# SCZwangxiao/video-ReTaKe

Measured on NVIDIA B200. Metric: 2048-frame DPSelect+PivotKV frames/s, higher is better.
Workload: dtype bf16

## Files before the change

include/rtk_b200.h:

```cpp
#ifndef RTK_B200_H_
#define RTK_B200_H_

#include <stddef.h>
#include <stdint.h>

#ifdef __cplusplus
extern "C" {
#endif

#define RTK_ABI_VERSION 3

#define RTK_E_BADARG      (-1)
#define RTK_E_ALIGN       (-2)
#define RTK_E_UNSUPPORTED (-3)
#define RTK_E_WORKSPACE   (-4)
#define RTK_E_DRIVER      (-5)

int         rtk_version(void);
const char* rtk_build_id(void);
const char* rtk_error_string(int code);
int         rtk_debug_key_elision(int on);
int64_t     rtk_launch_count(void);


int rtk_dpselect_dis(const void* x, int64_t T, int64_t N, int64_t C, int halo, float* dis, void* stream);

int rtk_dpselect_select(const float* dis, int64_t T, int64_t N, int64_t t, int sync,
                        int32_t* idx, uint8_t* mask, void* stream);

int rtk_dpselect_gather(const void* x, int64_t T, int64_t N, int64_t C, const int32_t* idx, int64_t t,
                        int sync, void* out, void* stream);

int rtk_dpselect_keyframe(const void* x, int64_t T, int64_t N, int64_t C, int64_t t, int sync, float* dis,
                          int32_t* idx, uint8_t* mask, void* out, void* stream);

int rtk_dpselect_gather_owned(const void* x_local, int64_t frames_local, int64_t frame_first, int64_t t0, int64_t t1,
                              int64_t N, int64_t C, const int32_t* idx, int64_t t, int sync, void* out, void* stream);

int rtk_gather_rows(const void* x, int64_t row_bytes, const int64_t* src_row, int64_t rows, void* out, void* stream);

size_t rtk_mallm_workspace_bytes(int64_t T, int64_t N, int64_t C, int hard);
int rtk_mallm_compress(const void* x, const void* sizes_in, int64_t T, int64_t N, int64_t C, int64_t t, int sync, int hard,
                       void* out, void* sizes_out, void* workspace, size_t workspace_bytes, void* stream);


int rtk_pivot_rope(const void* x, int64_t heads, int64_t L, int64_t D, int64_t stride_h, int64_t stride_l,
                   const void* cos, const void* sin, int n_pos, const int32_t* mrope_section_host,
                   float inv_scale2, int forward, void* out, int64_t out_stride_h, int64_t out_stride_l,
                   void* stream);

size_t rtk_pivot_score_workspace_bytes(int64_t H, int64_t L);

int rtk_pivot_score(const void* q, int64_t H, int64_t q_stride_h, int64_t q_stride_l,
                    const void* k, int64_t KVH, int64_t k_stride_h, int64_t k_stride_l,
                    int64_t L, int64_t D, void* head_scores, void* workspace, size_t workspace_bytes,
                    void* stream);

int rtk_pivot_select(const void* head_scores, int64_t KVH, int64_t L, const uint8_t* keymask, int64_t keep,
                     int32_t* keep_idx, void* score_out, void* stream);

int rtk_pivot_compact(const void* k, const void* v, int64_t KVH, int64_t L, int64_t D,
                      int64_t stride_h, int64_t stride_l, const int32_t* keep_idx, int64_t keep,
                      void* k_out, void* v_out, int64_t out_stride_h,
                      const int64_t* pos, int n_pos, int64_t* pos_out, int reforge, void* stream);

int rtk_kv_block_copy(int n_jobs, const void* const* src, void* const* dst, const int64_t* heads, const int64_t* rows,
                      const int64_t* src_stride_h, const int64_t* src_stride_l, const int64_t* dst_stride_h,
                      const int64_t* dst_stride_l, int64_t D, void* stream);

int rtk_pivot_rope_tables(const int64_t* pos, int n_pos, int64_t L, int64_t D, const float* inv_freq,
                          const int32_t* mrope_section_host, float attention_scaling, void* cos_out, void* sin_out,
                          void* stream);

typedef struct rtk_pivot_update_args {
    const void* q; int64_t H, q_stride_h, q_stride_l;
    const void* k; int64_t KVH, k_stride_h, k_stride_l;
    const void* v; int64_t v_stride_h, v_stride_l;
    int64_t k_stride_h_in, k_stride_l_in;
    int64_t L, D;
    const uint8_t* keymask;
    int64_t keep;
    int32_t reforge;
    int32_t n_pos;
    const int64_t* pos;
    const void* cos; const void* sin;
    const float* inv_freq;
    float attention_scaling, inv_scale2;
    int32_t mrope_section[3];
    int32_t skip_select;
    void* k_out; void* v_out; int64_t out_stride_h;
    int64_t* pos_out;
    int32_t* keep_idx;
    void* head_scores;
    void* workspace; size_t workspace_bytes;
    void* ev_score_begin; void* ev_score_end;
    int64_t pos_out_stride;
    int32_t skip_score;
    int32_t score_rows;
    int32_t xchg_world, xchg_rank;
    uint32_t xchg_epoch;
    void* xchg_scores[8];
    uint32_t* xchg_flags[8];
} rtk_pivot_update_args;

size_t rtk_pivot_update_workspace_bytes(int64_t H, int64_t KVH, int64_t L, int64_t D);
int rtk_pivot_update(const rtk_pivot_update_args* args, void* stream);

size_t rtk_pivot_update_batch_workspace_bytes(int64_t H, int64_t KVH, int64_t L, int64_t D, int64_t n_layers);
int rtk_pivot_update_batch(const rtk_pivot_update_args* layers, int64_t n_layers, void* workspace, size_t workspace_bytes,
                           void* stream);

#ifdef __cplusplus
}
#endif
#endif
```

video-retake_b200/csrc/pivot_misc.cu:

```cuda
#include <climits>

#include <stdlib.h>

#include "rtk_common.cuh"

namespace rtk {

struct RopeParams {
    int heads, L, D, n_pos, forward;
    long long stride_h, stride_l, out_stride_h, out_stride_l;
    int heads2;
    const __nv_bfloat16* x2;
    __nv_bfloat16* out2;
    long long stride_h2, stride_l2, out_stride_h2, out_stride_l2;
    int bound[6];
    float inv_scale2;
};

static bool mrope_bounds(int n_pos, const int32_t* sec, int64_t D, int bound[6]) {
    int acc = 0;
    for (int i = 0; i < 6; ++i) {
        acc += n_pos == 3 ? sec[i % 3] : 0;
        bound[i] = acc;
    }
    return n_pos != 3 || acc == D;
}

__device__ __forceinline__ int rope_pos_row(const RopeParams& p, int c) {
    if (p.n_pos == 1) return 0;
    int i = 0;
    while (i < 5 && c >= p.bound[i]) ++i;
    return i % 3;
}

__global__ void __launch_bounds__(256)
pivot_rope_table_kernel(const long long* __restrict__ pos, const float* __restrict__ inv_freq, RopeParams p, float scaling,
                        __nv_bfloat16* __restrict__ cos_t, __nv_bfloat16* __restrict__ sin_t) {
    pdl_enter();
    const int half = p.D >> 1;
    const long long total = (long long)p.L * p.D;
    for (long long i = (long long)blockIdx.x * blockDim.x + threadIdx.x; i < total; i += (long long)gridDim.x * blockDim.x) {
        const int c = (int)(i % p.D);
        const int l = (int)(i / p.D);
        const long long pv = pos[(size_t)rope_pos_row(p, c) * p.L + l];
        const float ang = inv_freq[c < half ? c : c - half] * (float)pv;
        cos_t[i] = __float2bfloat16_rn(cosf(ang) * scaling);
        sin_t[i] = __float2bfloat16_rn(sinf(ang) * scaling);
    }
}

__device__ __forceinline__ void rope_rotate_pair(float xa, float xb, float cosa, float sina, float cosb, float sinb, int forward,
                                                 float inv_scale2, __nv_bfloat16& oa, __nv_bfloat16& ob) {
    const float ta = round_bf16(xa * cosa), ra = round_bf16(-xb * sina);
    const float tb = round_bf16(xb * cosb), rb = round_bf16(xa * sinb);
    float ya, yb;
    if (forward) {
        ya = ta + ra;
        yb = tb + rb;
    } else {
        ya = round_bf16(ta - ra) * inv_scale2;
        yb = round_bf16(tb - rb) * inv_scale2;
    }
    oa = __float2bfloat16_rn(ya);
    ob = __float2bfloat16_rn(yb);
}

__device__ __forceinline__ void rope_table_entry(const RopeParams& p, const float* __restrict__ inv_freq, const long long* pv,
                                                 int c, float scaling, float& co, float& si) {
    const int half = p.D >> 1;
    const float ang = inv_freq[c < half ? c : c - half] * (float)pv[rope_pos_row(p, c)];
    co = __bfloat162float(__float2bfloat16_rn(cosf(ang) * scaling));
    si = __bfloat162float(__float2bfloat16_rn(sinf(ang) * scaling));
}

#ifndef RTK_UNROPE_TOK
#define RTK_UNROPE_TOK 2
#endif
constexpr int kUnropeTok = RTK_UNROPE_TOK;

__device__ __forceinline__ uint32_t sub_bf16x2_rn(uint32_t a, uint32_t b) {
    uint32_t d;
    asm("sub.rn.bf16x2 %0, %1, %2;" : "=r"(d) : "r"(a), "r"(b));
    return d;
}
__device__ __forceinline__ uint32_t add_bf16x2_rn(uint32_t a, uint32_t b) {
    uint32_t d;
    asm("add.rn.bf16x2 %0, %1, %2;" : "=r"(d) : "r"(a), "r"(b));
    return d;
}
__device__ __forceinline__ void unrotate_bf16x2(uint32_t xa, uint32_t xb, uint32_t cs, uint32_t sn, bool scale, float inv_scale2,
                                                uint32_t& oa, uint32_t& ob) {
    const uint32_t ta = mul_bf16x2_rn(xa, cs), ra = mul_bf16x2_rn(xb ^ 0x80008000u, sn);
    const uint32_t tb = mul_bf16x2_rn(xb, cs), rb = mul_bf16x2_rn(xa, sn);
    oa = sub_bf16x2_rn(ta, ra);
    ob = sub_bf16x2_rn(tb, rb);
    if (scale) {
        oa = scale_bf16x2_rn(oa, inv_scale2);
        ob = scale_bf16x2_rn(ob, inv_scale2);
    }
}

__device__ __forceinline__ void unrope_qk_body(const __nv_bfloat16* __restrict__ x, const long long* __restrict__ pos,
                                               const float* __restrict__ inv_freq, float scaling,
                                               __nv_bfloat16* __restrict__ out, const RopeParams& p) {
    __shared__ __align__(16) __nv_bfloat16 s_cos[kUnropeTok][128], s_sin[kUnropeTok][128];
    const int half = p.D >> 1;
    const int vec_per_row = half >> 3;
    const int ntask = (p.heads + p.heads2) * vec_per_row;
    const int tid = threadIdx.x;
    const bool scale = p.inv_scale2 != 1.0f;
    const int v0 = tid % vec_per_row, h0 = tid / vec_per_row;
    const bool second0 = h0 >= p.heads;
    const long long src_h0 = second0 ? (long long)(h0 - p.heads) * p.stride_h2 : (long long)h0 * p.stride_h;
    const long long src_l0 = second0 ? p.stride_l2 : p.stride_l;
    const __nv_bfloat16* src0 = (second0 ? p.x2 : x) + src_h0 + v0 * 8;
    for (int l0 = blockIdx.x * kUnropeTok; l0 < p.L; l0 += gridDim.x * kUnropeTok) {
        const int nl = min(kUnropeTok, p.L - l0);
        uint4 lo4[kUnropeTok], hi4[kUnropeTok];
        if (tid < ntask) {
#pragma unroll
            for (int t = 0; t < kUnropeTok; ++t) {
                if (t < nl) {
                    lo4[t] = *reinterpret_cast<const uint4*>(src0 + (l0 + t) * src_l0);
                    hi4[t] = *reinterpret_cast<const uint4*>(src0 + (l0 + t) * src_l0 + half);
                }
            }
        }
        for (int e = tid; e < nl * half; e += blockDim.x) {
            const int t = e / half, c = e - t * half;
            long long pv[3] = {0, 0, 0};
            for (int r = 0; r < p.n_pos; ++r) pv[r] = pos[(size_t)r * p.L + l0 + t];
            float co, si;
            rope_table_entry(p, inv_freq, pv, c, scaling, co, si);
            s_cos[t][c] = __float2bfloat16_rn(co);
            s_sin[t][c] = __float2bfloat16_rn(si);
        }
        __syncthreads();
#pragma unroll
        for (int t = 0; t < kUnropeTok; ++t) {
            if (t >= nl) break;
            const int l = l0 + t;
            for (int task = tid; task < ntask; task += blockDim.x) {
                const int v = task % vec_per_row, h = task / vec_per_row;
                const int c0 = v * 8;
                const bool second = h >= p.heads;
                const __nv_bfloat16* src = second ? p.x2 + (h - p.heads) * p.stride_h2 + l * p.stride_l2 : x + h * p.stride_h + l * p.stride_l;
                __nv_bfloat16* dst = second ? p.out2 + (h - p.heads) * p.out_stride_h2 + l * p.out_stride_l2
                                            : out + h * p.out_stride_h + l * p.out_stride_l;
                uint4 a4 = lo4[t], b4 = hi4[t];
                if (task != tid) {
                    a4 = *reinterpret_cast<const uint4*>(src + c0);
                    b4 = *reinterpret_cast<const uint4*>(src + c0 + half);
                }
                const uint4 cs = *reinterpret_cast<const uint4*>(&s_cos[t][c0]);
                const uint4 sn = *reinterpret_cast<const uint4*>(&s_sin[t][c0]);
                uint4 ol4, oh4;
                unrotate_bf16x2(a4.x, b4.x, cs.x, sn.x, scale, p.inv_scale2, ol4.x, oh4.x);
                unrotate_bf16x2(a4.y, b4.y, cs.y, sn.y, scale, p.inv_scale2, ol4.y, oh4.y);
                unrotate_bf16x2(a4.z, b4.z, cs.z, sn.z, scale, p.inv_scale2, ol4.z, oh4.z);
                unrotate_bf16x2(a4.w, b4.w, cs.w, sn.w, scale, p.inv_scale2, ol4.w, oh4.w);
                *reinterpret_cast<uint4*>(dst + c0) = ol4;
                *reinterpret_cast<uint4*>(dst + c0 + half) = oh4;
            }
        }
        __syncthreads();
    }
}

struct BatchLayers {
    const __nv_bfloat16* q[kMaxBatchLayers];
    const __nv_bfloat16* k[kMaxBatchLayers];
    const __nv_bfloat16* k_in[kMaxBatchLayers];
    const __nv_bfloat16* v[kMaxBatchLayers];
    __nv_bfloat16* qu[kMaxBatchLayers];
    __nv_bfloat16* ku[kMaxBatchLayers];
    const long long* pos[kMaxBatchLayers];
    const uint8_t* keymask[kMaxBatchLayers];
    __nv_bfloat16* k_out[kMaxBatchLayers];
    __nv_bfloat16* v_out[kMaxBatchLayers];
    long long* pos_out[kMaxBatchLayers];
    int32_t* keep_idx[kMaxBatchLayers];
    const __nv_bfloat16* head_scores[kMaxBatchLayers];
    long long q_stride_h[kMaxBatchLayers], q_stride_l[kMaxBatchLayers];
    long long kin_stride_h[kMaxBatchLayers], kin_stride_l[kMaxBatchLayers];
    long long k_stride_h[kMaxBatchLayers], k_stride_l[kMaxBatchLayers];
    long long v_stride_h[kMaxBatchLayers], v_stride_l[kMaxBatchLayers];
    long long out_stride_h[kMaxBatchLayers], pos_out_stride[kMaxBatchLayers];
};

__global__ void __launch_bounds__(256)
pivot_unrope_qk_batch_kernel(const __grid_constant__ BatchLayers t, const float* __restrict__ inv_freq, float scaling, RopeParams p) {
    pdl_enter();
    const int layer = blockIdx.y;
    p.stride_h = t.q_stride_h[layer]; p.stride_l = t.q_stride_l[layer];
    p.x2 = t.k_in[layer]; p.out2 = t.ku[layer];
    p.stride_h2 = t.kin_stride_h[layer]; p.stride_l2 = t.kin_stride_l[layer];
    unrope_qk_body(t.q[layer], t.pos[layer], inv_freq, scaling, t.qu[layer], p);
}

__global__ void __launch_bounds__(256)
pivot_rope_kernel(const __nv_bfloat16* __restrict__ x, const __nv_bfloat16* __restrict__ cos_t,
                  const __nv_bfloat16* __restrict__ sin_t, __nv_bfloat16* __restrict__ out, RopeParams p) {
    pdl_enter();
    const int half = p.D >> 1;
    const int vec_per_row = half >> 3;
    const long long total = (long long)(p.heads + p.heads2) * p.L * vec_per_row;
    for (long long i = (long long)blockIdx.x * blockDim.x + threadIdx.x; i < total; i += (long long)gridDim.x * blockDim.x) {
        const int v = (int)(i % vec_per_row);
        const long long hl = i / vec_per_row;
        const int l = (int)(hl % p.L);
        const int h = (int)(hl / p.L);
        const int c0 = v * 8;
        const bool second = h >= p.heads;
        const __nv_bfloat16* src = second ? p.x2 + (h - p.heads) * p.stride_h2 + l * p.stride_l2 : x + h * p.stride_h + l * p.stride_l;
        __nv_bfloat16* dst = second ? p.out2 + (h - p.heads) * p.out_stride_h2 + l * p.out_stride_l2
                                    : out + h * p.out_stride_h + l * p.out_stride_l;
        uint4 lo4 = *reinterpret_cast<const uint4*>(src + c0);
        uint4 hi4 = *reinterpret_cast<const uint4*>(src + c0 + half);
        const __nv_bfloat16* xl = reinterpret_cast<const __nv_bfloat16*>(&lo4);
        const __nv_bfloat16* xh = reinterpret_cast<const __nv_bfloat16*>(&hi4);
        uint4 ol4, oh4;
        __nv_bfloat16* ol = reinterpret_cast<__nv_bfloat16*>(&ol4);
        __nv_bfloat16* oh = reinterpret_cast<__nv_bfloat16*>(&oh4);
        const int rowa0 = rope_pos_row(p, c0), rowa1 = rope_pos_row(p, c0 + 7);
        const int rowb0 = rope_pos_row(p, c0 + half), rowb1 = rope_pos_row(p, c0 + half + 7);
        uint4 ca4, sa4, cb4, sb4;
        __nv_bfloat16* cav = reinterpret_cast<__nv_bfloat16*>(&ca4);
        __nv_bfloat16* sav = reinterpret_cast<__nv_bfloat16*>(&sa4);
        __nv_bfloat16* cbv = reinterpret_cast<__nv_bfloat16*>(&cb4);
        __nv_bfloat16* sbv = reinterpret_cast<__nv_bfloat16*>(&sb4);
        if (rowa0 == rowa1 && rowb0 == rowb1) {
            const size_t ia = ((size_t)rowa0 * p.L + l) * p.D + c0, ib = ((size_t)rowb0 * p.L + l) * p.D + c0 + half;
            ca4 = __ldg(reinterpret_cast<const uint4*>(cos_t + ia));
            sa4 = __ldg(reinterpret_cast<const uint4*>(sin_t + ia));
            cb4 = __ldg(reinterpret_cast<const uint4*>(cos_t + ib));
            sb4 = __ldg(reinterpret_cast<const uint4*>(sin_t + ib));
        } else {
#pragma unroll
            for (int e = 0; e < 8; ++e) {
                const int ca = c0 + e, cb = c0 + e + half;
                const size_t ia = ((size_t)rope_pos_row(p, ca) * p.L + l) * p.D + ca;
                const size_t ib = ((size_t)rope_pos_row(p, cb) * p.L + l) * p.D + cb;
                cav[e] = cos_t[ia]; sav[e] = sin_t[ia]; cbv[e] = cos_t[ib]; sbv[e] = sin_t[ib];
            }
        }
#pragma unroll
        for (int e = 0; e < 8; ++e)
            rope_rotate_pair(__bfloat162float(xl[e]), __bfloat162float(xh[e]), __bfloat162float(cav[e]), __bfloat162float(sav[e]),
                             __bfloat162float(cbv[e]), __bfloat162float(sbv[e]), p.forward, p.inv_scale2, ol[e], oh[e]);
        *reinterpret_cast<uint4*>(dst + c0) = ol4;
        *reinterpret_cast<uint4*>(dst + c0 + half) = oh4;
    }
}

bool key_elision_enabled();

struct KeyElide {
    const uint8_t* keymask[kMaxBatchLayers];
    int32_t* slot[kMaxBatchLayers];
    const __nv_bfloat16* k[kMaxBatchLayers];
    long long k_stride_h[kMaxBatchLayers], k_stride_l[kMaxBatchLayers];
    __nv_bfloat16* kc[kMaxBatchLayers];
    int32_t* n_keys;
    int L, KVH, D;
};

__global__ void __launch_bounds__(1024)
pivot_keymask_scan_kernel(const __grid_constant__ KeyElide e) {
    pdl_enter();
    __shared__ int wsum[32];
    const int layer = blockIdx.x, tid = threadIdx.x, lane = tid & 31, warp = tid >> 5;
    const uint8_t* __restrict__ m = e.keymask[layer];
    int32_t* __restrict__ slot = e.slot[layer];
    const int per = (e.L + 1023) / 1024;
    const int beg = min(tid * per, e.L), end = min(beg + per, e.L);
    int cnt = 0;
    for (int i = beg; i < end; ++i) cnt += !(m && m[i]);
    int inc = cnt;
#pragma unroll
    for (int o = 1; o < 32; o <<= 1) {
        const int n = __shfl_up_sync(0xffffffffu, inc, o);
        if (lane >= o) inc += n;
    }
    if (lane == 31) wsum[warp] = inc;
    __syncthreads();
    if (warp == 0) {
        const int w = wsum[lane];
        int winc = w;
#pragma unroll
        for (int o = 1; o < 32; o <<= 1) {
            const int n = __shfl_up_sync(0xffffffffu, winc, o);
            if (lane >= o) winc += n;
        }
        wsum[lane] = winc - w;
        if (lane == 31) e.n_keys[layer] = winc;
    }
    __syncthreads();
    int base = wsum[warp] + inc - cnt;
    for (int i = beg; i < end; ++i) slot[i] = (m && m[i]) ? -1 : base++;
}

__global__ void __launch_bounds__(256)
pivot_keys_compact_kernel(const __grid_constant__ KeyElide e) {
    pdl_enter();
    const int layer = blockIdx.y;
    const int vpr = e.D >> 3;
    const long long total = (long long)e.L * e.KVH * vpr;
    const int32_t* __restrict__ slot = e.slot[layer];
    for (long long i = (long long)blockIdx.x * blockDim.x + threadIdx.x; i < total; i += (long long)gridDim.x * blockDim.x) {
        const int v = (int)(i % vpr);
        const long long lh = i / vpr;
        const int h = (int)(lh % e.KVH);
        const int l = (int)(lh / e.KVH);
        const int sl = slot[l];
        if (sl < 0) continue;
        const uint4 w = __ldg(reinterpret_cast<const uint4*>(e.k[layer] + h * e.k_stride_h[layer] + l * e.k_stride_l[layer] + v * 8));
        *reinterpret_cast<uint4*>(e.kc[layer] + ((size_t)sl * e.KVH + h) * e.D + v * 8) = w;
    }
}

static int key_elide_prepare(KeyElide& ke, int n, ScoreBatch& sb, cudaStream_t st) {
    RTK_LAUNCH_PDL(pivot_keymask_scan_kernel, (unsigned)n, 1024, 0, st, ke);
    const long long total = (long long)ke.L * ke.KVH * (ke.D >> 3);
    long long gx = (total + 255) / 256;
    if (gx > 148 * 8) gx = 148 * 8;
    RTK_LAUNCH_PDL(pivot_keys_compact_kernel, dim3((unsigned)gx, (unsigned)n), 256, 0, st, ke);
    for (int i = 0; i < n; ++i) {
        sb.kc[i] = ke.kc[i];
        sb.slot[i] = ke.slot[i];
    }
    sb.n_keys = ke.n_keys;
    return 0;
}

static size_t key_elide_bytes(int64_t KVH, int64_t L, int64_t D) {
    return (((size_t)KVH * L * D * 2 + 255) & ~(size_t)255) + (((size_t)L * 4 + 255) & ~(size_t)255);
}

constexpr int kSelThreads = 1024;

__device__ void block_select_top(const uint32_t* keys, int L, int keep, int32_t* out_idx, int* sh ,
                                 int low_bit ) {
    const int tid = threadIdx.x, lane = tid & 31, warp = tid >> 5;
    const int per = (L + kSelThreads - 1) / kSelThreads;
    const int beg = min(tid * per, L), end = min(beg + per, L);
    uint32_t prefix = 0;
    for (int bit = 31; bit >= low_bit; --bit) {
        const uint32_t cand = prefix | (1u << bit);
        int cnt = 0;
        for (int i = beg; i < end; ++i) cnt += (keys[i] >= cand);
        cnt = __reduce_add_sync(0xffffffffu, cnt);
        int* buf = sh + 40 + 32 * (bit & 1);
        if (lane == 0) buf[warp] = cnt;
        __syncthreads();
        const int total = __reduce_add_sync(0xffffffffu, buf[lane]);
        if (total >= keep) prefix = cand;
    }
    __syncthreads();
    if (low_bit > 0 && (!(prefix & 0x80000000u) || (prefix >> low_bit) == (0xffffffffu >> low_bit)))
        prefix |= (1u << low_bit) - 1u;
    int gt = 0, eq = 0;
    for (int i = beg; i < end; ++i) { gt += (keys[i] > prefix); eq += (keys[i] == prefix); }
    auto block_excl_scan = [&](int v, int& total) {
        int inc = v;
#pragma unroll
        for (int o = 1; o < 32; o <<= 1) {
            const int n = __shfl_up_sync(0xffffffffu, inc, o);
            if (lane >= o) inc += n;
        }
        __syncthreads();
        if (lane == 31) sh[1 + warp] = inc;
        __syncthreads();
        if (warp == 0) {
            int w = sh[1 + lane], winc = w;
#pragma unroll
            for (int o = 1; o < 32; o <<= 1) {
                const int n = __shfl_up_sync(0xffffffffu, winc, o);
                if (lane >= o) winc += n;
            }
            sh[1 + lane] = winc - w;
            if (lane == 31) sh[33] = winc;
        }
        __syncthreads();
        total = sh[33];
        return sh[1 + warp] + inc - v;
    };
    int gt_total, eq_total;
    const int gt_before = block_excl_scan(gt, gt_total);
    const int eq_before = block_excl_scan(eq, eq_total);
    const int need = keep - gt_total;
    const int eq_taken_before = min(eq_before, need);
    int slot = gt_before + eq_taken_before;
    int eq_seen = eq_before;
    for (int i = beg; i < end; ++i) {
        const uint32_t k = keys[i];
        bool take = k > prefix;
        if (k == prefix) { take = eq_seen < need; ++eq_seen; }
        if (take) out_idx[slot++] = i;
    }
}

__device__ __forceinline__ void pivot_select_body(const __nv_bfloat16* __restrict__ head_scores, int KVH, int L,
                                                  const uint8_t* __restrict__ keymask, int keep, int32_t* __restrict__ keep_idx,
                                                  __nv_bfloat16* __restrict__ score_out, const long long* __restrict__ tpos,
                                                  long long* __restrict__ tmin_out) {
    extern __shared__ __align__(128) uint8_t smem[];
    uint32_t* keys = reinterpret_cast<uint32_t*>(smem);
    int* sh = reinterpret_cast<int*>(smem + (size_t)L * 4);
    const float rcp = 1.0f / (float)KVH;
    for (int i = threadIdx.x; i < L; i += blockDim.x) {
        float v[4] = {0.f, 0.f, 0.f, 0.f};
        for (int j = 0; j < KVH; ++j) v[j & 3] += __bfloat162float(head_scores[(size_t)j * L + i]);
        const __nv_bfloat16 s = __float2bfloat16_rn((((v[0] + v[1]) + v[2]) + v[3]) * rcp);
        if (score_out) score_out[i] = s;
        const float f = (keymask && keymask[i]) ? 1.0f : __bfloat162float(s);
        keys[i] = f32_to_ordered(f);
    }
    __syncthreads();
    block_select_top(keys, L, keep, keep_idx, sh, 16);
    if (tmin_out) {
        __syncthreads();
        long long* smin = reinterpret_cast<long long*>((reinterpret_cast<uintptr_t>(sh) + 7) & ~(uintptr_t)7);
        long long mn = LLONG_MAX;
        for (int j = threadIdx.x; j < keep; j += blockDim.x) mn = min(mn, tpos[keep_idx[j]]);
#pragma unroll
        for (int o = 16; o > 0; o >>= 1) mn = min(mn, __shfl_xor_sync(0xffffffffu, mn, o));
        if ((threadIdx.x & 31) == 0) smin[threadIdx.x >> 5] = mn;
        __syncthreads();
        if (threadIdx.x == 0) {
            for (int w = 1; w < (int)(blockDim.x >> 5); ++w) mn = min(mn, smin[w]);
            *tmin_out = mn;
        }
    }
}

__device__ __forceinline__ void st_release_sys(uint32_t* p, uint32_t v) {
    asm volatile("st.release.sys.global.u32 [%0], %1;" ::"l"(p), "r"(v) : "memory");
}
__device__ __forceinline__ uint32_t ld_acquire_sys(const uint32_t* p) {
    uint32_t v;
    asm volatile("ld.acquire.sys.global.u32 %0, [%1];" : "=r"(v) : "l"(p) : "memory");
    return v;
}
__device__ __forceinline__ unsigned long long globaltimer_ns() {
    unsigned long long t;
    asm volatile("mov.u64 %0, %%globaltimer;" : "=l"(t));
    return t;
}
__device__ __forceinline__ void xchg_wait(const uint32_t* flags, int n, uint32_t epoch, unsigned long long timeout_ns) {
    if ((int)threadIdx.x < n) {
        const unsigned long long t0 = globaltimer_ns();
        while (ld_acquire_sys(flags + threadIdx.x) != epoch) {
            __nanosleep(64);
            if (timeout_ns && globaltimer_ns() - t0 > timeout_ns) __trap();
        }
    }
    __syncthreads();
}
struct XchgPutBatch {
    const __nv_bfloat16* src[kMaxBatchLayers];
    __nv_bfloat16* dst[kMaxBatchLayers][8];
    long long n;
    int world, rank;
};
__global__ void __launch_bounds__(1024)
pivot_xchg_put_batch_kernel(const __grid_constant__ XchgPutBatch p) {
    pdl_enter();
    const int layer = blockIdx.x;
    const __nv_bfloat16* src = p.src[layer];
    for (int r = 0; r < p.world; ++r) {
        if (r == p.rank) continue;
        __nv_bfloat16* dst = p.dst[layer][r];
        if ((((uintptr_t)src | (uintptr_t)dst) & 15u) == 0) {
            const long long nv = p.n >> 3;
            for (long long i = threadIdx.x; i < nv; i += blockDim.x)
                reinterpret_cast<uint4*>(dst)[i] = reinterpret_cast<const uint4*>(src)[i];
            for (long long i = (nv << 3) + threadIdx.x; i < p.n; i += blockDim.x) dst[i] = src[i];
        } else {
            for (long long i = threadIdx.x; i < p.n; i += blockDim.x) dst[i] = src[i];
        }
    }
    __threadfence_system();
}
struct XchgFlags {
    uint32_t* flags[8];
    int world, rank;
    uint32_t epoch;
};
__global__ void __launch_bounds__(32)
pivot_xchg_flag_kernel(XchgFlags p) {
    pdl_enter();
    __threadfence_system();
    if ((int)threadIdx.x < p.world) st_release_sys(p.flags[threadIdx.x] + p.rank, p.epoch);
}

__global__ void __launch_bounds__(kSelThreads)
pivot_select_kernel(const __nv_bfloat16* __restrict__ head_scores, int KVH, int L, const uint8_t* __restrict__ keymask,
                    int keep, int32_t* __restrict__ keep_idx, __nv_bfloat16* __restrict__ score_out) {
    pdl_enter();
    pivot_select_body(head_scores, KVH, L, keymask, keep, keep_idx, score_out, nullptr, nullptr);
}

__global__ void __launch_bounds__(kSelThreads)
pivot_select_batch_kernel(const __grid_constant__ BatchLayers t, int KVH, int L, int keep, int reforge, long long* __restrict__ tmin,
                          const uint32_t* __restrict__ wait_flags, int wait_n, uint32_t wait_epoch, unsigned long long wait_ns) {
    pdl_enter();
    if (wait_flags) xchg_wait(wait_flags, wait_n, wait_epoch, wait_ns);
    const int layer = blockIdx.x;
    pivot_select_body(t.head_scores[layer], KVH, L, t.keymask[layer], keep, t.keep_idx[layer], nullptr,
                      reforge ? t.pos[layer] : nullptr, reforge ? tmin + layer : nullptr);
}

struct CompactParams {
    int KVH, L, D, keep, n_pos, reforge;
    long long stride_h, stride_l, out_stride_h;
    long long v_stride_h, v_stride_l;
    long long pos_out_stride;
    float ratio;
};

__global__ void __launch_bounds__(256)
pivot_compact_kernel(const __nv_bfloat16* __restrict__ k, const __nv_bfloat16* __restrict__ v,
                     const int32_t* __restrict__ keep_idx, __nv_bfloat16* __restrict__ k_out,
                     __nv_bfloat16* __restrict__ v_out, const long long* __restrict__ pos,
                     long long* __restrict__ pos_out, CompactParams p) {
    pdl_enter();
    if (blockIdx.x == gridDim.x - 1) {
        if (!pos) return;
        __shared__ long long smin[32];
        const int tid = threadIdx.x, lane = tid & 31, warp = tid >> 5;
        for (int r = p.reforge ? 1 : 0; r < p.n_pos; ++r)
            for (int j = tid; j < p.keep; j += blockDim.x) pos_out[(size_t)r * p.keep + j] = pos[(size_t)r * p.L + keep_idx[j]];
        if (!p.reforge) return;
        long long mn = LLONG_MAX;
        for (int j = tid; j < p.keep; j += blockDim.x) mn = min(mn, pos[keep_idx[j]]);
#pragma unroll
        for (int o = 16; o > 0; o >>= 1) mn = min(mn, __shfl_xor_sync(0xffffffffu, mn, o));
        if (lane == 0) smin[warp] = mn;
        __syncthreads();
        mn = smin[0];
        for (int w = 1; w < (int)(blockDim.x >> 5); ++w) mn = min(mn, smin[w]);
        for (int j = tid; j < p.keep; j += blockDim.x) {
            const float d = (float)(pos[keep_idx[j]] - mn);
            pos_out[j] = mn + (long long)(d * p.ratio);
        }
        return;
    }
    const int vec_per_row = p.D >> 3;
    const long long total = (long long)p.KVH * p.keep * vec_per_row;
    const long long nthreads = (long long)(gridDim.x - 1) * blockDim.x;
    for (long long i = (long long)blockIdx.x * blockDim.x + threadIdx.x; i < total; i += nthreads) {
        const int c = (int)(i % vec_per_row);
        const long long hj = i / vec_per_row;
        const int j = (int)(hj % p.keep);
        const int h = (int)(hj / p.keep);
        const int src_row = keep_idx[j];
        const size_t so = (size_t)h * p.stride_h + (size_t)src_row * p.stride_l + (size_t)c * 8;
        const size_t sv = (size_t)h * p.v_stride_h + (size_t)src_row * p.v_stride_l + (size_t)c * 8;
        const size_t dof = (size_t)h * p.out_stride_h + (size_t)j * p.D + (size_t)c * 8;
        if (k) *reinterpret_cast<uint4*>(k_out + dof) = __ldg(reinterpret_cast<const uint4*>(k + so));
        if (v) *reinterpret_cast<uint4*>(v_out + dof) = __ldg(reinterpret_cast<const uint4*>(v + sv));
    }
}

__device__ __forceinline__ void compact_rope_body(const __nv_bfloat16* __restrict__ k, const __nv_bfloat16* __restrict__ v,
                                                  const int32_t* __restrict__ keep_idx, __nv_bfloat16* __restrict__ k_out,
                                                  __nv_bfloat16* __restrict__ v_out, const long long* __restrict__ pos,
                                                  long long* __restrict__ pos_out, const long long* __restrict__ tmin,
                                                  const float* __restrict__ inv_freq, float scaling, const CompactParams& p,
                                                  const RopeParams& rp, int rotate) {
    __shared__ float s_cos[256], s_sin[256];
    __shared__ long long s_pos[3];
    const int j = blockIdx.x, tid = threadIdx.x;
    const int src_row = keep_idx[j];
    if (pos && tid < p.n_pos) {
        long long pv = pos[(size_t)tid * p.L + src_row];
        if (p.reforge && tid == 0) {
            const long long mn = *tmin;
            pv = mn + (long long)((float)(pv - mn) * p.ratio);
        }
        pos_out[(size_t)tid * p.pos_out_stride + j] = pv;
        s_pos[tid] = pv;
    }
    const int vec_per_row = p.D >> 3;
    for (int t = tid; t < p.KVH * vec_per_row; t += blockDim.x) {
        const int c = t % vec_per_row, h = t / vec_per_row;
        const size_t dof = (size_t)h * p.out_stride_h + (size_t)j * p.D + (size_t)c * 8;
        *reinterpret_cast<uint4*>(v_out + dof) =
            __ldg(reinterpret_cast<const uint4*>(v + (size_t)h * p.v_stride_h + (size_t)src_row * p.v_stride_l + (size_t)c * 8));
        if (!rotate)
            *reinterpret_cast<uint4*>(k_out + dof) =
                __ldg(reinterpret_cast<const uint4*>(k + (size_t)h * p.stride_h + (size_t)src_row * p.stride_l + (size_t)c * 8));
    }
    if (!rotate) return;
    __syncthreads();
    if (tid < p.D) rope_table_entry(rp, inv_freq, s_pos, tid, scaling, s_cos[tid], s_sin[tid]);
    __syncthreads();
    const int half = p.D >> 1, hv = half >> 3;
    for (int t = tid; t < p.KVH * hv; t += blockDim.x) {
        const int c0 = (t % hv) * 8, h = t / hv;
        const __nv_bfloat16* src = k + (size_t)h * p.stride_h + (size_t)src_row * p.stride_l;
        __nv_bfloat16* dst = k_out + (size_t)h * p.out_stride_h + (size_t)j * p.D;
        uint4 lo4 = *reinterpret_cast<const uint4*>(src + c0);
        uint4 hi4 = *reinterpret_cast<const uint4*>(src + c0 + half);
        const __nv_bfloat16* xl = reinterpret_cast<const __nv_bfloat16*>(&lo4);
        const __nv_bfloat16* xh = reinterpret_cast<const __nv_bfloat16*>(&hi4);
        uint4 ol4, oh4;
        __nv_bfloat16* ol = reinterpret_cast<__nv_bfloat16*>(&ol4);
        __nv_bfloat16* oh = reinterpret_cast<__nv_bfloat16*>(&oh4);
#pragma unroll
        for (int e = 0; e < 8; ++e)
            rope_rotate_pair(__bfloat162float(xl[e]), __bfloat162float(xh[e]), s_cos[c0 + e], s_sin[c0 + e], s_cos[c0 + half + e],
                             s_sin[c0 + half + e], 1, 1.0f, ol[e], oh[e]);
        *reinterpret_cast<uint4*>(dst + c0) = ol4;
        *reinterpret_cast<uint4*>(dst + c0 + half) = oh4;
    }
}

__global__ void __launch_bounds__(128)
pivot_compact_rope_batch_kernel(const __grid_constant__ BatchLayers t, const long long* __restrict__ tmin,
                                const float* __restrict__ inv_freq, float scaling, CompactParams p, RopeParams rp, int rotate) {
    pdl_enter();
    const int layer = blockIdx.y;
    p.stride_h = t.k_stride_h[layer]; p.stride_l = t.k_stride_l[layer];
    p.v_stride_h = t.v_stride_h[layer]; p.v_stride_l = t.v_stride_l[layer];
    p.out_stride_h = t.out_stride_h[layer];
    p.pos_out_stride = t.pos_out_stride[layer];
    compact_rope_body(t.k[layer], t.v[layer], t.keep_idx[layer], t.k_out[layer], t.v_out[layer], t.pos[layer], t.pos_out[layer],
                      tmin + layer, inv_freq, scaling, p, rp, rotate);
}

struct CopyJobs {
    int n;
    const __nv_bfloat16* src[4];
    __nv_bfloat16* dst[4];
    int heads[4], rows[4];
    long long src_stride_h[4], src_stride_l[4], dst_stride_h[4], dst_stride_l[4];
    long long vec_end[4];
    int D;
};

__global__ void __launch_bounds__(256)
kv_block_copy_kernel(CopyJobs j) {
    pdl_enter();
    const int vpr = j.D >> 3;
    const long long total = j.vec_end[j.n - 1];
    for (long long i = (long long)blockIdx.x * blockDim.x + threadIdx.x; i < total; i += (long long)gridDim.x * blockDim.x) {
        int k = 0;
        while (i >= j.vec_end[k]) ++k;
        const long long li = i - (k ? j.vec_end[k - 1] : 0);
        const int c = (int)(li % vpr);
        const long long hr = li / vpr;
        const int r = (int)(hr % j.rows[k]);
        const int h = (int)(hr / j.rows[k]);
        const uint4 v = __ldg(reinterpret_cast<const uint4*>(j.src[k] + h * j.src_stride_h[k] + r * j.src_stride_l[k] + c * 8));
        *reinterpret_cast<uint4*>(j.dst[k] + h * j.dst_stride_h[k] + r * j.dst_stride_l[k] + c * 8) = v;
    }
}

long long g_launches = 0;
static int g_key_elision = -1;
bool key_elision_enabled() {
    if (g_key_elision < 0) {
        const char* e = getenv("RTK_NO_KEY_ELISION");
        g_key_elision = (e && e[0] == '1') ? 0 : 1;
    }
    return g_key_elision != 0;
}
unsigned long long xchg_timeout_ns() {
    static const unsigned long long ns = [] {
        const char* e = getenv("RTK_XCHG_TIMEOUT_S");
        const double s = (e && e[0]) ? atof(e) : 120.0;
        return s > 0.0 ? (unsigned long long)(s * 1e9) : 0ull;
    }();
    return ns;
}
bool pdl_enabled() {
    static const bool on = [] {
        const char* e = getenv("RTK_NO_PDL");
        return !(e && e[0] && e[0] != '0');
    }();
    return on;
}

}

using namespace rtk;

extern "C" int rtk_version(void) { return RTK_ABI_VERSION; }

extern "C" int rtk_debug_key_elision(int on) {
    const int prev = rtk::key_elision_enabled() ? 1 : 0;
    if (on >= 0) rtk::g_key_elision = on ? 1 : 0;
    return prev;
}

#ifndef RTK_BUILD_ID
#define RTK_BUILD_ID "unknown"
#endif
extern "C" const char* rtk_build_id(void) { return RTK_BUILD_ID; }

extern "C" int64_t rtk_launch_count(void) { return (int64_t)rtk::g_launches; }

extern "C" const char* rtk_error_string(int code) {
    if (code == 0) return "ok";
    if (code > 0) return cudaGetErrorString((cudaError_t)code);
    switch (code) {
        case RTK_E_BADARG: return "rtk: bad argument (null pointer or non-positive size)";
        case RTK_E_ALIGN: return "rtk: pointer or stride not 16-byte aligned";
        case RTK_E_UNSUPPORTED: return "rtk: shape outside the supported envelope";
        case RTK_E_WORKSPACE: return "rtk: workspace too small";
        case RTK_E_DRIVER: return "rtk: cuTensorMapEncodeTiled unavailable or failed";
        default: return "rtk: unknown error";
    }
}

static int rope_launch(const void* x, const void* cos, const void* sin, void* out, const RopeParams& p, cudaStream_t st) {
    const long long total = (long long)(p.heads + p.heads2) * p.L * (p.D / 16);
    long long grid = (total + 255) / 256;
    if (grid > 148 * 16) grid = 148 * 16;
    RTK_LAUNCH_PDL(pivot_rope_kernel, (unsigned)grid, 256, 0, st, (const __nv_bfloat16*)x, (const __nv_bfloat16*)cos, (const __nv_bfloat16*)sin, (__nv_bfloat16*)out, p);
    return 0;
}

extern "C" int rtk_pivot_rope(const void* x, int64_t heads, int64_t L, int64_t D, int64_t stride_h, int64_t stride_l,
                              const void* cos, const void* sin, int n_pos, const int32_t* mrope_section_host,
                              float inv_scale2, int forward, void* out, int64_t out_stride_h, int64_t out_stride_l,
                              void* stream) {
    RTK_NVTX("rtk_pivot_rope");
    if (!x || !cos || !sin || !out || heads < 1 || L < 1 || D < 16) return RTK_E_BADARG;
    if (D % 16 != 0 || (n_pos != 1 && n_pos != 3)) return RTK_E_UNSUPPORTED;
    if (n_pos == 3 && !mrope_section_host) return RTK_E_BADARG;
    if ((((uintptr_t)x | (uintptr_t)out) & 15u) != 0) return RTK_E_ALIGN;
    if ((stride_h | stride_l | out_stride_h | out_stride_l) % 8 != 0) return RTK_E_ALIGN;
    RopeParams p;
    p.heads = (int)heads; p.L = (int)L; p.D = (int)D; p.n_pos = n_pos; p.forward = forward;
    p.stride_h = stride_h; p.stride_l = stride_l; p.out_stride_h = out_stride_h; p.out_stride_l = out_stride_l;
    p.inv_scale2 = inv_scale2;
    p.heads2 = 0; p.x2 = nullptr; p.out2 = nullptr;
    p.stride_h2 = p.stride_l2 = p.out_stride_h2 = p.out_stride_l2 = 0;
    if (!mrope_bounds(n_pos, mrope_section_host, D, p.bound)) return RTK_E_UNSUPPORTED;
    return rope_launch(x, cos, sin, out, p, (cudaStream_t)stream);
}

extern "C" int rtk_pivot_select(const void* head_scores, int64_t KVH, int64_t L, const uint8_t* keymask, int64_t keep,
                                int32_t* keep_idx, void* score_out, void* stream) {
    RTK_NVTX("rtk_pivot_select");
    if (!head_scores || !keep_idx || KVH < 1 || L < 1 || keep < 1 || keep > L) return RTK_E_BADARG;
    if (L > 16384) return RTK_E_UNSUPPORTED;
    const size_t smem = (size_t)L * 4 + 112 * 4;
    cudaError_t e = cudaFuncSetAttribute(pivot_select_kernel, cudaFuncAttributeMaxDynamicSharedMemorySize, (int)smem);
    if (e != cudaSuccess) return (int)e;
    RTK_LAUNCH_PDL(pivot_select_kernel, 1, kSelThreads, smem, (cudaStream_t)stream, (const __nv_bfloat16*)head_scores, (int)KVH,
                   (int)L, keymask, (int)keep, keep_idx, (__nv_bfloat16*)score_out);
    return 0;
}

extern "C" int rtk_pivot_compact(const void* k, const void* v, int64_t KVH, int64_t L, int64_t D, int64_t stride_h,
                                 int64_t stride_l, const int32_t* keep_idx, int64_t keep, void* k_out, void* v_out,
                                 int64_t out_stride_h, const int64_t* pos, int n_pos, int64_t* pos_out, int reforge,
                                 void* stream) {
    RTK_NVTX("rtk_pivot_compact");
    if ((!k && !v) || !keep_idx || (k && !k_out) || (v && !v_out) || KVH < 1 || L < 1 || D < 8 || keep < 1 || keep > L)
        return RTK_E_BADARG;
    if (pos && (!pos_out || n_pos < 1)) return RTK_E_BADARG;
    if (D % 8 != 0) return RTK_E_UNSUPPORTED;
    if ((((uintptr_t)k | (uintptr_t)v | (uintptr_t)k_out | (uintptr_t)v_out) & 15u) != 0) return RTK_E_ALIGN;
    if ((stride_h | stride_l | out_stride_h) % 8 != 0) return RTK_E_ALIGN;
    CompactParams p;
    p.KVH = (int)KVH; p.L = (int)L; p.D = (int)D; p.keep = (int)keep; p.n_pos = n_pos; p.reforge = reforge;
    p.stride_h = stride_h; p.stride_l = stride_l; p.out_stride_h = out_stride_h;
    p.v_stride_h = stride_h; p.v_stride_l = stride_l;
    p.pos_out_stride = keep;
    p.ratio = (float)((double)keep / (double)L);
    const long long total = KVH * keep * (D / 8);
    long long grid = (total + 255) / 256;
    if (grid > 148 * 8) grid = 148 * 8;
    RTK_LAUNCH_PDL(pivot_compact_kernel, (unsigned)(grid + 1), 256, 0, (cudaStream_t)stream,  (const __nv_bfloat16*)k, (const __nv_bfloat16*)v, keep_idx, (__nv_bfloat16*)k_out, (__nv_bfloat16*)v_out, (const long long*)pos, (long long*)pos_out, p);
    return 0;
}

extern "C" int rtk_pivot_rope_tables(const int64_t* pos, int n_pos, int64_t L, int64_t D, const float* inv_freq,
                                     const int32_t* mrope_section_host, float attention_scaling, void* cos_out,
                                     void* sin_out, void* stream) {
    RTK_NVTX("rtk_pivot_rope_tables");
    if (!pos || !inv_freq || !cos_out || !sin_out || L < 1 || D < 2) return RTK_E_BADARG;
    if (D % 2 != 0 || (n_pos != 1 && n_pos != 3)) return RTK_E_UNSUPPORTED;
    if (n_pos == 3 && !mrope_section_host) return RTK_E_BADARG;
    RopeParams p;
    p.heads = 1; p.L = (int)L; p.D = (int)D; p.n_pos = n_pos; p.forward = 0;
    p.stride_h = p.stride_l = p.out_stride_h = p.out_stride_l = 0;
    p.heads2 = 0; p.x2 = nullptr; p.out2 = nullptr;
    p.stride_h2 = p.stride_l2 = p.out_stride_h2 = p.out_stride_l2 = 0;
    p.inv_scale2 = 1.0f;
    if (!mrope_bounds(n_pos, mrope_section_host, D, p.bound)) return RTK_E_UNSUPPORTED;
    long long grid = (L * D + 255) / 256;
    if (grid > 148 * 8) grid = 148 * 8;
    RTK_LAUNCH_PDL(pivot_rope_table_kernel, (unsigned)grid, 256, 0, (cudaStream_t)stream,  (const long long*)pos, inv_freq, p, attention_scaling, (__nv_bfloat16*)cos_out, (__nv_bfloat16*)sin_out);
    return 0;
}

static size_t align256(size_t x) { return (x + 255) & ~(size_t)255; }

extern "C" size_t rtk_pivot_update_batch_workspace_bytes(int64_t H, int64_t KVH, int64_t L, int64_t D, int64_t n_layers) {
    if (H < 1 || KVH < 1 || L < 1 || D < 1 || n_layers < 1) return 0;
    const size_t n = (size_t)(n_layers < kMaxBatchLayers ? n_layers : kMaxBatchLayers);
    return align256(rtk_pivot_score_workspace_bytes(H * (int64_t)n, L)) +
           n * (align256((size_t)H * L * D * 2) + align256((size_t)KVH * L * D * 2)) + align256(n * sizeof(long long)) + 256 +
           n * key_elide_bytes(KVH, L, D) + 256;
}

extern "C" size_t rtk_pivot_update_workspace_bytes(int64_t H, int64_t KVH, int64_t L, int64_t D) {
    return rtk_pivot_update_batch_workspace_bytes(H, KVH, L, D, 1);
}

#ifndef RTK_UNROT_TOKEN_MAJOR
#define RTK_UNROT_TOKEN_MAJOR 1
#endif

static int pivot_update_group(const rtk_pivot_update_args* a, int n, char* ws, cudaStream_t st) {
    const rtk_pivot_update_args& a0 = a[0];
    const int64_t H = a0.H, KVH = a0.KVH, L = a0.L, D = a0.D;
    const bool reforge = a0.reforge != 0;
    const int64_t uq_sh = RTK_UNROT_TOKEN_MAJOR ? D : L * D, uq_sl = RTK_UNROT_TOKEN_MAJOR ? H * D : D;
    const int64_t uk_sh = RTK_UNROT_TOKEN_MAJOR ? D : L * D, uk_sl = RTK_UNROT_TOKEN_MAJOR ? KVH * D : D;
    void* score_ws = ws;                ws += align256(rtk_pivot_score_workspace_bytes(H * n, L));
    char* qu0 = ws;                     ws += (size_t)n * align256((size_t)H * L * D * 2);
    char* ku0 = ws;                     ws += (size_t)n * align256((size_t)KVH * L * D * 2);
    long long* tmin = (long long*)ws;   ws += align256((size_t)n * sizeof(long long)) + 256;
    char* kc0 = ws;                     ws += (size_t)n * align256((size_t)KVH * L * D * 2);
    char* slot0 = ws;                   ws += (size_t)n * align256((size_t)L * 4);
    int32_t* nkeys_ws = (int32_t*)ws;

    BatchLayers t = {};
    ScoreBatch sb = {};
    sb.n = n; sb.H = H; sb.KVH = KVH; sb.L = L; sb.D = D;
    for (int i = 0; i < kMaxBatchLayers; ++i) {
        const rtk_pivot_update_args& x = a[i < n ? i : 0];
        char* qu = qu0 + (size_t)(i < n ? i : 0) * align256((size_t)H * L * D * 2);
        char* ku = ku0 + (size_t)(i < n ? i : 0) * align256((size_t)KVH * L * D * 2);
        t.q[i] = (const __nv_bfloat16*)x.q;       t.q_stride_h[i] = x.q_stride_h;     t.q_stride_l[i] = x.q_stride_l;
        t.k_in[i] = (const __nv_bfloat16*)x.k;    t.kin_stride_h[i] = x.k_stride_h;   t.kin_stride_l[i] = x.k_stride_l;
        t.qu[i] = (__nv_bfloat16*)qu;             t.ku[i] = (__nv_bfloat16*)ku;
        t.k[i] = reforge ? (const __nv_bfloat16*)ku : (const __nv_bfloat16*)x.k;
        t.k_stride_h[i] = reforge ? uk_sh : x.k_stride_h;
        t.k_stride_l[i] = reforge ? uk_sl : x.k_stride_l;
        t.v[i] = (const __nv_bfloat16*)x.v;       t.v_stride_h[i] = x.v_stride_h;     t.v_stride_l[i] = x.v_stride_l;
        t.pos[i] = (const long long*)x.pos;       t.keymask[i] = x.keymask;
        t.k_out[i] = (__nv_bfloat16*)x.k_out;     t.v_out[i] = (__nv_bfloat16*)x.v_out;
        t.out_stride_h[i] = x.out_stride_h;
        t.pos_out[i] = (long long*)x.pos_out;     t.pos_out_stride[i] = x.pos_out_stride > 0 ? x.pos_out_stride : x.keep;
        t.keep_idx[i] = x.keep_idx;               t.head_scores[i] = (const __nv_bfloat16*)x.head_scores;
        if (i < n) {
            sb.q[i] = reforge ? (const void*)qu : x.q;
            sb.k[i] = reforge ? (const void*)ku : x.k;
            sb.q_stride_h[i] = reforge ? uq_sh : x.q_stride_h;   sb.q_stride_l[i] = reforge ? uq_sl : x.q_stride_l;
            sb.k_stride_h[i] = reforge ? uk_sh : x.k_stride_h;   sb.k_stride_l[i] = reforge ? uk_sl : x.k_stride_l;
            sb.head_scores[i] = x.head_scores;
        }
    }
    RopeParams rp = {};
    rp.heads = (int)H; rp.L = (int)L; rp.D = (int)D; rp.n_pos = a0.n_pos; rp.forward = 0;
    rp.out_stride_h = uq_sh; rp.out_stride_l = uq_sl;
    rp.heads2 = (int)KVH; rp.out_stride_h2 = uk_sh; rp.out_stride_l2 = uk_sl;
    rp.inv_scale2 = a0.inv_scale2;
    mrope_bounds(a0.n_pos, a0.mrope_section, D, rp.bound);
    const bool xchg = a0.xchg_world > 1;
    const int64_t score_rows = a0.score_rows > 0 ? a0.score_rows : KVH;
    if (reforge && !a0.skip_score) {
        if (a0.inv_freq) {
            RTK_LAUNCH_PDL(pivot_unrope_qk_batch_kernel, dim3((unsigned)((L + kUnropeTok - 1) / kUnropeTok), (unsigned)n), 256, 0, st, t, a0.inv_freq,
                           a0.attention_scaling, rp);
        } else {
            rp.stride_h = a0.q_stride_h; rp.stride_l = a0.q_stride_l;
            rp.x2 = t.k_in[0]; rp.out2 = t.ku[0]; rp.stride_h2 = a0.k_stride_h; rp.stride_l2 = a0.k_stride_l;
            const int rc = rope_launch(a0.q, a0.cos, a0.sin, t.qu[0], rp, st);
            if (rc) return rc;
        }
    }
    if (!a0.skip_score) {
        bool any_mask = false;
        for (int i = 0; i < n; ++i) any_mask = any_mask || a[i].keymask != nullptr;
        if (any_mask && key_elision_enabled()) {
            KeyElide ke = {};
            ke.L = (int)L; ke.KVH = (int)KVH; ke.D = (int)D; ke.n_keys = nkeys_ws;
            for (int i = 0; i < kMaxBatchLayers; ++i) {
                const int j = i < n ? i : 0;
                ke.keymask[i] = a[j].keymask;
                ke.slot[i] = (int32_t*)(slot0 + (size_t)j * align256((size_t)L * 4));
                ke.k[i] = t.k[j]; ke.k_stride_h[i] = t.k_stride_h[j]; ke.k_stride_l[i] = t.k_stride_l[j];
                ke.kc[i] = (__nv_bfloat16*)(kc0 + (size_t)j * align256((size_t)KVH * L * D * 2));
            }
            int rc = key_elide_prepare(ke, n, sb, st);
            if (rc) return rc;
        }
        if (a0.ev_score_begin) cudaEventRecord((cudaEvent_t)a0.ev_score_begin, st);
        int rc = pivot_score_batch(sb, score_ws, rtk_pivot_score_workspace_bytes(H * n, L), st);
        if (rc) return rc;
        if (a0.ev_score_end) cudaEventRecord((cudaEvent_t)a0.ev_score_end, st);
    }
    if (a0.skip_select) {
        if (xchg) {
            XchgPutBatch xp = {};
            xp.n = (long long)KVH * L; xp.world = a0.xchg_world; xp.rank = a0.xchg_rank;
            for (int i = 0; i < n; ++i) {
                xp.src[i] = (const __nv_bfloat16*)a[i].head_scores;
                for (int r = 0; r < a0.xchg_world; ++r)
                    xp.dst[i][r] = (__nv_bfloat16*)a[i].xchg_scores[r] + (size_t)a0.xchg_rank * KVH * L;
            }
            RTK_LAUNCH_PDL(pivot_xchg_put_batch_kernel, (unsigned)n, 1024, 0, st, xp);
            XchgFlags xf = {};
            xf.world = a0.xchg_world; xf.rank = a0.xchg_rank; xf.epoch = a0.xchg_epoch;
            for (int r = 0; r < a0.xchg_world; ++r) xf.flags[r] = a0.xchg_flags[r];
            RTK_LAUNCH_PDL(pivot_xchg_flag_kernel, 1, 32, 0, st, xf);
        }
        return 0;
    }
    {
        const size_t smem = (size_t)L * 4 + 112 * 4;
        cudaError_t e = cudaFuncSetAttribute(pivot_select_batch_kernel, cudaFuncAttributeMaxDynamicSharedMemorySize, (int)smem);
        if (e != cudaSuccess) return (int)e;
        RTK_LAUNCH_PDL(pivot_select_batch_kernel, (unsigned)n, kSelThreads, smem, st, t, (int)score_rows, (int)L, (int)a0.keep,
                       reforge ? 1 : 0, tmin, (const uint32_t*)(xchg ? a0.xchg_flags[a0.xchg_rank] : nullptr),
                       xchg ? a0.xchg_world : 0, a0.xchg_epoch, xchg_timeout_ns());
    }
    {
        CompactParams p = {};
        p.KVH = (int)KVH; p.L = (int)L; p.D = (int)D; p.keep = (int)a0.keep; p.n_pos = a0.pos ? a0.n_pos : 0; p.reforge = a0.reforge;
        p.ratio = (float)((double)a0.keep / (double)L);
        RopeParams rq = {};
        rq.D = (int)D; rq.n_pos = a0.n_pos; rq.L = (int)a0.keep;
        for (int i = 0; i < 6; ++i) rq.bound[i] = rp.bound[i];
        RTK_LAUNCH_PDL(pivot_compact_rope_batch_kernel, dim3((unsigned)a0.keep, (unsigned)n), 128, 0, st, t, (const long long*)tmin,
                       a0.inv_freq, a0.attention_scaling, p, rq, (reforge && a0.inv_freq) ? 1 : 0);
    }
    return 0;
}

static int update_check(const rtk_pivot_update_args* layers, int64_t n, const void* workspace, size_t workspace_bytes) {
    if (!layers || n < 1 || !workspace) return RTK_E_BADARG;
    const rtk_pivot_update_args& a0 = layers[0];
    const bool scores = !a0.skip_score, selects = !a0.skip_select, xchg = a0.xchg_world > 1;
    if (!scores && !selects) return RTK_E_BADARG;
    if (a0.H < 1 || a0.KVH < 1 || a0.L < 1 || (selects && (a0.keep < 1 || a0.keep > a0.L))) return RTK_E_BADARG;
    if (a0.L > 16384 || a0.D % 16 != 0 || a0.D > 256) return RTK_E_UNSUPPORTED;
    if (scores && ((a0.D != 64 && a0.D != 128) || a0.H % a0.KVH != 0 || a0.H > 256)) return RTK_E_UNSUPPORTED;
    if (xchg) {
        if (n > kMaxBatchLayers) return RTK_E_UNSUPPORTED;
        if (a0.xchg_world > 8 || a0.xchg_rank < 0 || a0.xchg_rank >= a0.xchg_world || (scores && selects)) return RTK_E_BADARG;
    }
    if (a0.reforge && !a0.inv_freq && n > 1) return RTK_E_UNSUPPORTED;
    int bound[6];
    if (a0.reforge && (scores || a0.inv_freq) && !mrope_bounds(a0.n_pos, a0.mrope_section, a0.D, bound)) return RTK_E_UNSUPPORTED;
    if (((uintptr_t)workspace & 255u) != 0) return RTK_E_ALIGN;
    if (workspace_bytes < rtk_pivot_update_batch_workspace_bytes(a0.H, a0.KVH, a0.L, a0.D, n)) return RTK_E_WORKSPACE;
    for (int64_t i = 0; i < n; ++i) {
        const rtk_pivot_update_args& x = layers[i];
        if (!x.q || !x.k || !x.v || !x.k_out || !x.v_out || !x.keep_idx || !x.head_scores) return RTK_E_BADARG;
        if (x.H != a0.H || x.KVH != a0.KVH || x.L != a0.L || x.D != a0.D || x.keep != a0.keep || x.reforge != a0.reforge ||
            x.n_pos != a0.n_pos || x.inv_freq != a0.inv_freq || x.attention_scaling != a0.attention_scaling ||
            x.inv_scale2 != a0.inv_scale2 || x.skip_select != a0.skip_select || x.skip_score != a0.skip_score ||
            x.score_rows != a0.score_rows || x.xchg_world != a0.xchg_world || x.xchg_rank != a0.xchg_rank ||
            x.xchg_epoch != a0.xchg_epoch || (x.pos == nullptr) != (a0.pos == nullptr))
            return RTK_E_UNSUPPORTED;
        for (int j = 0; j < 3; ++j)
            if (x.mrope_section[j] != a0.mrope_section[j]) return RTK_E_UNSUPPORTED;
        if (x.reforge && (!x.pos || !x.pos_out || (!x.inv_freq && (!x.cos || !x.sin)))) return RTK_E_BADARG;
        if (xchg) {
            for (int r = 0; r < a0.xchg_world; ++r)
                if (!x.xchg_scores[r] || !a0.xchg_flags[r]) return RTK_E_BADARG;
            const char* own = (const char*)x.xchg_scores[a0.xchg_rank];
            if (a0.skip_score && (const char*)x.head_scores != own) return RTK_E_BADARG;
            if (a0.skip_select && (const char*)x.head_scores != own + (size_t)a0.xchg_rank * a0.KVH * a0.L * 2) return RTK_E_BADARG;
        }
        if (x.pos && (selects || x.reforge) && (!x.pos_out || x.n_pos < 1 || x.n_pos > 3)) return RTK_E_BADARG;
        uintptr_t ptrs = 0;
        int64_t strides = 0;
        if (scores) {
            ptrs |= (uintptr_t)x.q;
            strides |= x.q_stride_h | x.q_stride_l;
        }
        if (scores || !x.reforge) {
            ptrs |= (uintptr_t)x.k;
            strides |= x.k_stride_h | x.k_stride_l;
        }
        if (selects) {
            ptrs |= (uintptr_t)x.v | (uintptr_t)x.k_out | (uintptr_t)x.v_out;
            strides |= x.v_stride_h | x.v_stride_l | x.out_stride_h;
        }
        if ((ptrs & 15u) != 0 || strides % 8 != 0) return RTK_E_ALIGN;
    }
    return 0;
}

extern "C" int rtk_pivot_update(const rtk_pivot_update_args* a, void* stream) {
    RTK_NVTX("rtk_pivot_update");
    if (!a) return RTK_E_BADARG;
    const int rc = update_check(a, 1, a->workspace, a->workspace_bytes);
    if (rc) return rc;
    return pivot_update_group(a, 1, (char*)a->workspace, (cudaStream_t)stream);
}

extern "C" int rtk_pivot_update_batch(const rtk_pivot_update_args* layers, int64_t n_layers, void* workspace,
                                      size_t workspace_bytes, void* stream) {
    RTK_NVTX("rtk_pivot_update_batch");
    int rc = update_check(layers, n_layers, workspace, workspace_bytes);
    if (rc) return rc;
    for (int64_t i = 0; i < n_layers; i += kMaxBatchLayers) {
        const int n = (int)((n_layers - i) < kMaxBatchLayers ? (n_layers - i) : kMaxBatchLayers);
        rc = pivot_update_group(layers + i, n, (char*)workspace, (cudaStream_t)stream);
        if (rc) return rc;
    }
    return 0;
}

extern "C" int rtk_kv_block_copy(int n_jobs, const void* const* src, void* const* dst, const int64_t* heads, const int64_t* rows,
                                 const int64_t* src_stride_h, const int64_t* src_stride_l, const int64_t* dst_stride_h,
                                 const int64_t* dst_stride_l, int64_t D, void* stream) {
    RTK_NVTX("rtk_kv_block_copy");
    if (n_jobs < 1 || n_jobs > 4 || !src || !dst || !heads || !rows || D < 8) return RTK_E_BADARG;
    if (D % 8 != 0) return RTK_E_UNSUPPORTED;
    CopyJobs j;
    j.n = n_jobs;
    j.D = (int)D;
    long long acc = 0;
    for (int k = 0; k < n_jobs; ++k) {
        if (!src[k] || !dst[k] || heads[k] < 1 || rows[k] < 0) return RTK_E_BADARG;
        if ((((uintptr_t)src[k] | (uintptr_t)dst[k]) & 15u) != 0) return RTK_E_ALIGN;
        if ((src_stride_h[k] | src_stride_l[k] | dst_stride_h[k] | dst_stride_l[k]) % 8 != 0) return RTK_E_ALIGN;
        j.src[k] = (const __nv_bfloat16*)src[k];
        j.dst[k] = (__nv_bfloat16*)dst[k];
        j.heads[k] = (int)heads[k];
        j.rows[k] = (int)rows[k];
        j.src_stride_h[k] = src_stride_h[k]; j.src_stride_l[k] = src_stride_l[k];
        j.dst_stride_h[k] = dst_stride_h[k]; j.dst_stride_l[k] = dst_stride_l[k];
        acc += heads[k] * rows[k] * (D / 8);
        j.vec_end[k] = acc;
    }
    for (int k = n_jobs; k < 4; ++k) j.vec_end[k] = acc;
    if (acc == 0) return 0;
    long long grid = (acc + 255) / 256;
    if (grid > 148 * 8) grid = 148 * 8;
    RTK_LAUNCH_PDL(kv_block_copy_kernel, (unsigned)grid, 256, 0, (cudaStream_t)stream, j);
    return 0;
}
```

video-retake_b200/csrc/pivot_score.cu:

```cuda
#include <cuda.h>

#include "rtk_common.cuh"

namespace rtk {

constexpr int kTile = 128;
constexpr int kHeadDim = 128;
constexpr int kPair = 2;
constexpr int kStages = 2;
constexpr int kASlots = 2;
constexpr int kAccBufs = 4;
constexpr int kStatSlots = kStages + kAccBufs;
constexpr uint32_t kTileBytes = kTile * kHeadDim * 2;
constexpr uint32_t kHalfBytes = kTile * 64 * 2;

struct ScoreSmem {
    static constexpr uint32_t a_tile = 0;
    static constexpr uint32_t b_ring = kASlots * kPair * kTileBytes;
    static constexpr uint32_t stats = b_ring + kStages * kTileBytes;
    static constexpr uint32_t merge = stats + kStatSlots * kTile * 4;
    static constexpr uint32_t bars = merge + 4 * kTile * 2 * 4;
    static constexpr uint32_t n_bars = 4 + 2 * kStages + 2 * kAccBufs + kStatSlots;
    static constexpr uint32_t tmem_ptr = bars + n_bars * 8;
    static constexpr uint32_t total = tmem_ptr + 16;
};

__device__ __forceinline__ void tmem_alloc(uint32_t smem_dst, uint32_t ncols) {
    asm volatile("tcgen05.alloc.cta_group::1.sync.aligned.shared::cta.b32 [%0], %1;" ::"r"(smem_dst), "r"(ncols) : "memory");
    asm volatile("tcgen05.relinquish_alloc_permit.cta_group::1.sync.aligned;" ::: "memory");
}
__device__ __forceinline__ void tmem_dealloc(uint32_t taddr, uint32_t ncols) {
    asm volatile("tcgen05.dealloc.cta_group::1.sync.aligned.b32 %0, %1;" ::"r"(taddr), "r"(ncols) : "memory");
}
__device__ __forceinline__ void tc_fence_before() { asm volatile("tcgen05.fence::before_thread_sync;" ::: "memory"); }
__device__ __forceinline__ void tc_fence_after() { asm volatile("tcgen05.fence::after_thread_sync;" ::: "memory"); }
__device__ __forceinline__ void tc_commit(uint32_t bar) {
    asm volatile("tcgen05.commit.cta_group::1.mbarrier::arrive::one.shared::cluster.b64 [%0];" ::"r"(bar) : "memory");
}
__device__ __forceinline__ void umma_bf16(uint32_t tmem_d, uint64_t adesc, uint64_t bdesc, uint32_t idesc, uint32_t accum) {
    asm volatile(
        "{\n\t.reg .pred p;\n\t"
        "setp.ne.b32 p, %4, 0;\n\t"
        "tcgen05.mma.cta_group::1.kind::f16 [%0], %1, %2, %3, p;\n\t}"
        ::"r"(tmem_d), "l"(adesc), "l"(bdesc), "r"(idesc), "r"(accum)
        : "memory");
}
__device__ __forceinline__ void tmem_ld_wait() { asm volatile("tcgen05.wait::ld.sync.aligned;" ::: "memory"); }
__device__ __forceinline__ void tmem_ld64(uint32_t taddr, uint32_t (&r)[64]) {
    asm volatile(
        "tcgen05.ld.sync.aligned.32x32b.x64.b32 "
        "{%0, %1, %2, %3, %4, %5, %6, %7, %8, %9, %10, %11, %12, %13, %14, %15, "
        "%16, %17, %18, %19, %20, %21, %22, %23, %24, %25, %26, %27, %28, %29, %30, %31, "
        "%32, %33, %34, %35, %36, %37, %38, %39, %40, %41, %42, %43, %44, %45, %46, %47, "
        "%48, %49, %50, %51, %52, %53, %54, %55, %56, %57, %58, %59, %60, %61, %62, %63}, [%64];"
        : "=r"(r[0]), "=r"(r[1]), "=r"(r[2]), "=r"(r[3]), "=r"(r[4]), "=r"(r[5]), "=r"(r[6]), "=r"(r[7]),
          "=r"(r[8]), "=r"(r[9]), "=r"(r[10]), "=r"(r[11]), "=r"(r[12]), "=r"(r[13]), "=r"(r[14]), "=r"(r[15]),
          "=r"(r[16]), "=r"(r[17]), "=r"(r[18]), "=r"(r[19]), "=r"(r[20]), "=r"(r[21]), "=r"(r[22]), "=r"(r[23]),
          "=r"(r[24]), "=r"(r[25]), "=r"(r[26]), "=r"(r[27]), "=r"(r[28]), "=r"(r[29]), "=r"(r[30]), "=r"(r[31]),
          "=r"(r[32]), "=r"(r[33]), "=r"(r[34]), "=r"(r[35]), "=r"(r[36]), "=r"(r[37]), "=r"(r[38]), "=r"(r[39]),
          "=r"(r[40]), "=r"(r[41]), "=r"(r[42]), "=r"(r[43]), "=r"(r[44]), "=r"(r[45]), "=r"(r[46]), "=r"(r[47]),
          "=r"(r[48]), "=r"(r[49]), "=r"(r[50]), "=r"(r[51]), "=r"(r[52]), "=r"(r[53]), "=r"(r[54]), "=r"(r[55]),
          "=r"(r[56]), "=r"(r[57]), "=r"(r[58]), "=r"(r[59]), "=r"(r[60]), "=r"(r[61]), "=r"(r[62]), "=r"(r[63])
        : "r"(taddr)
        : "memory");
}
__device__ __forceinline__ void add_bf16_pair(float& acc_lo, float& acc_hi, uint32_t packed) {
    asm("{\n\t.reg .b16 lo, hi;\n\t"
        "mov.b32 {lo, hi}, %2;\n\t"
        "add.rn.f32.bf16 %0, lo, %0;\n\t"
        "add.rn.f32.bf16 %1, hi, %1;\n\t}"
        : "+f"(acc_lo), "+f"(acc_hi)
        : "r"(packed));
}

__device__ __forceinline__ void tma_load_3d(uint32_t dst, const CUtensorMap* map, int c0, int c1, int c2, uint32_t bar) {
    asm volatile(
        "cp.async.bulk.tensor.3d.shared::cluster.global.tile.mbarrier::complete_tx::bytes [%0], [%1, {%3, %4, %5}], [%2];"
        ::"r"(dst), "l"(reinterpret_cast<uint64_t>(map)), "r"(bar), "r"(c0), "r"(c1), "r"(c2)
        : "memory");
}
__device__ __forceinline__ float ex2f(float x) {
    float y;
    asm("ex2.approx.ftz.f32 %0, %1;" : "=f"(y) : "f"(x));
    return y;
}
__device__ __forceinline__ float lg2f(float x) {
    float y;
    asm("lg2.approx.ftz.f32 %0, %1;" : "=f"(y) : "f"(x));
    return y;
}

__device__ __forceinline__ uint64_t umma_desc_sw128(uint32_t smem_addr) {
    return (uint64_t)((smem_addr & 0x3ffffu) >> 4) | ((uint64_t)1 << 16) | ((uint64_t)(1024 >> 4) << 32) |
           ((uint64_t)1 << 46) | ((uint64_t)2 << 61);
}
constexpr uint32_t kIdesc = (1u << 4) | (1u << 7) | (1u << 10) | ((uint32_t)(kTile >> 3) << 17) | ((uint32_t)(kTile >> 4) << 24);

template <int NL>
struct ScoreMaps {
    CUtensorMap q[NL], k[NL];
    CUtensorMap kc[NL];
};

struct ScoreParams {
    int H, G, L, nt;
    int Hl;
    int n_atoms;
    int q_dim1_is_l, k_dim1_is_l;
    float inv_sqrt_d;
    const int32_t* n_keys;
    int kc_dim1_is_l;
    float2* ml_part;
    float* stats;
    float* colsum_part;
};

constexpr float kLog2e = 1.4426950408889634f;

__device__ __forceinline__ uint64_t pk2(float lo, float hi) {
    uint64_t d;
    asm("mov.b64 %0, {%1, %2};" : "=l"(d) : "f"(lo), "f"(hi));
    return d;
}
__device__ __forceinline__ void upk2(uint64_t v, float& lo, float& hi) {
    asm("mov.b64 {%0, %1}, %2;" : "=f"(lo), "=f"(hi) : "l"(v));
}
__device__ __forceinline__ uint64_t mul2(uint64_t a, uint64_t b) {
    uint64_t d;
    asm("mul.rn.f32x2 %0, %1, %2;" : "=l"(d) : "l"(a), "l"(b));
    return d;
}
__device__ __forceinline__ uint64_t fma2(uint64_t a, uint64_t b, uint64_t c) {
    uint64_t d;
    asm("fma.rn.f32x2 %0, %1, %2, %3;" : "=l"(d) : "l"(a), "l"(b), "l"(c));
    return d;
}
__device__ __forceinline__ uint64_t add2(uint64_t a, uint64_t b) {
    uint64_t d;
    asm("add.rn.f32x2 %0, %1, %2;" : "=l"(d) : "l"(a), "l"(b));
    return d;
}

__device__ __forceinline__ void mbar_wait_feeder(uint32_t bar, uint32_t parity) {
    while (!mbar_try_wait(bar, parity)) {
    }
}

__device__ __forceinline__ float round_bf16_inplace(float a) {
    uint32_t d;
    asm("cvt.rn.bf16x2.f32 %0, %1, %2;" : "=r"(d) : "f"(a), "f"(0.f));
    return __uint_as_float(d);
}

__device__ __forceinline__ uint64_t logit_chain2(uint32_t r0, uint32_t r1, uint64_t inv2) {
    float t0, t1;
    upk2(mul2(pk2(round_bf16_inplace(__uint_as_float(r0)), round_bf16_inplace(__uint_as_float(r1))), inv2), t0, t1);
    return pk2(round_bf16_inplace(t0), round_bf16_inplace(t1));
}
__device__ __forceinline__ float logit_chain1(float acc, float inv) { return round_bf16(round_bf16(acc) * inv); }

__device__ __forceinline__ uint64_t ex2_mufu2(uint64_t x2) {
    float x0, x1;
    upk2(x2, x0, x1);
    return pk2(ex2f(x0), ex2f(x1));
}

struct SoftmaxState {
    float m = -INFINITY;
    uint64_t acc = 0;
    float c0 = 0.f, c1 = 0.f;
};

template <int PASS>
__device__ __forceinline__ void softmax_cols(uint32_t (&r)[64], int valid, SoftmaxState& st, const float* cq, float inv,
                                             uint64_t inv2, uint64_t l2e2) {
    constexpr int NC = 64;
    if (PASS == 1) {
        if (valid < NC) {
#pragma unroll
            for (int i = 0; i < NC; ++i)
                if (i >= valid) r[i] = 0xff800000u;
        }
        float mx = fmaxf(fmaxf(__uint_as_float(r[0]), __uint_as_float(r[1])), __uint_as_float(r[2]));
#pragma unroll
        for (int i = 3; i < NC - 1; i += 2) mx = fmaxf(fmaxf(mx, __uint_as_float(r[i])), __uint_as_float(r[i + 1]));
        mx = fmaxf(mx, __uint_as_float(r[NC - 1]));
        const float mn = fmaxf(st.m, logit_chain1(mx, inv));
        if (!(mn > -INFINITY)) return;
        const float mm = mn * kLog2e;
        const float sc = ex2f(fmaf(st.m, kLog2e, -mm));
        st.acc = mul2(st.acc, pk2(sc, sc));
        st.m = mn;
        const uint64_t nmm = pk2(-mm, -mm);
#pragma unroll
        for (int i = 0; i < NC; i += 4) {
            st.acc = add2(st.acc, ex2_mufu2(fma2(logit_chain2(r[i], r[i + 1], inv2), l2e2, nmm)));
            st.acc = add2(st.acc, ex2_mufu2(fma2(logit_chain2(r[i + 2], r[i + 3], inv2), l2e2, nmm)));
        }
    } else {
#pragma unroll
        for (int i = 0; i < NC; i += 4) {
            const float4 cc = *reinterpret_cast<const float4*>(cq + i);
            float e0, e1, e2, e3;
            upk2(ex2_mufu2(fma2(logit_chain2(r[i], r[i + 1], inv2), l2e2, pk2(-cc.x, -cc.y))), e0, e1);
            upk2(ex2_mufu2(fma2(logit_chain2(r[i + 2], r[i + 3], inv2), l2e2, pk2(-cc.z, -cc.w))), e2, e3);
            add_bf16_pair(st.c0, st.c1, pack_bf16x2_rn(e0, e1));
            add_bf16_pair(st.c0, st.c1, pack_bf16x2_rn(e2, e3));
        }
    }
}

struct TileRange {
    int g, g1, Gl;
    int nt;
    int nt_a, nta;
    int layer, n_layers, Hl, geff;
    const int32_t* n_keys;
    __device__ __forceinline__ void set_layer_range() {
        nt_a = n_keys ? (n_keys[layer] + kTile - 1) / kTile : nt;
        nta = (nt_a + kPair - 1) / kPair;
        Gl = Hl * nta * nt;
        int ge = Gl / ((nt + 1) / 2);
        ge = ge < 1 ? 1 : (ge > (int)gridDim.x ? (int)gridDim.x : ge);
        geff = ge;
        if ((int)blockIdx.x < geff) {
            g = (int)((unsigned)Gl * blockIdx.x / (unsigned)geff);
            g1 = (int)((unsigned)Gl * (blockIdx.x + 1) / (unsigned)geff);
        } else {
            g = g1 = 0;
        }
    }
    __device__ __forceinline__ bool next_cta_reaches_end_of(int ul) const {
        return (int)((unsigned)Gl * (blockIdx.x + 2) / (unsigned)geff) >= (ul + 1) * nt;
    }
    __device__ __forceinline__ TileRange(int H, int Hl_, int nt_, const int32_t* n_keys_) : nt(nt_), layer(0), Hl(Hl_), n_keys(n_keys_) {
        n_layers = H / Hl_;
        set_layer_range();
    }
    __device__ __forceinline__ bool next(int& ul, int& tb0, int& tb1) {
        while (g >= g1) {
            if (++layer >= n_layers) return false;
            set_layer_range();
        }
        ul = g / nt;
        tb0 = g - ul * nt;
        const int left = g1 - g;
        tb1 = (left < nt - tb0) ? tb0 + left : nt;
        g += tb1 - tb0;
        return true;
    }
};

constexpr int kGroups = 4;
constexpr int kSoftmaxWarps = 4 * kGroups;
constexpr int kScoreThreads2 = (2 + kSoftmaxWarps) * 32;
constexpr int kTileArrivals = 8;

template <int PASS, int NL>
__global__ void __launch_bounds__(kScoreThreads2, 1)
pivot_score_kernel(const __grid_constant__ ScoreMaps<NL> maps, ScoreParams prm) {
    if (RTK_PDL_EARLY_SCORE) pdl_trigger();
    extern __shared__ __align__(1024) uint8_t smem_raw[];
    const uint32_t base = (smem_u32(smem_raw) + 1023u) & ~1023u;
    uint8_t* smem = smem_raw + (base - smem_u32(smem_raw));
    const int warp = threadIdx.x >> 5, lane = threadIdx.x & 31;

    const uint32_t bar0 = base + ScoreSmem::bars;
    auto a_full = [&](int i) { return bar0 + 8 * i; };
    auto a_empty = [&](int i) { return bar0 + 16 + 8 * i; };
    auto b_full = [&](int s) { return bar0 + 32 + 8 * s; };
    auto b_empty = [&](int s) { return bar0 + 32 + 8 * (kStages + s); };
    auto t_full = [&](int b) { return bar0 + 32 + 8 * (2 * kStages + b); };
    auto t_empty = [&](int b) { return bar0 + 32 + 8 * (2 * kStages + kAccBufs + b); };
    auto st_full = [&](int i) { return bar0 + 32 + 8 * (2 * kStages + 2 * kAccBufs + i); };

    if (threadIdx.x == 0) {
        for (int i = 0; i < 2; ++i) { mbar_init(a_full(i), 1); mbar_init(a_empty(i), 1); }
        for (int s = 0; s < kStages; ++s) { mbar_init(b_full(s), 1); mbar_init(b_empty(s), 1); }
        for (int b = 0; b < kAccBufs; ++b) { mbar_init(t_full(b), 1); mbar_init(t_empty(b), kTileArrivals); }
        for (int i = 0; i < kStatSlots; ++i) mbar_init(st_full(i), 1);
        fence_mbar_init();
    }
    if (warp == 1) tmem_alloc(base + ScoreSmem::tmem_ptr, 512);
    tc_fence_before();
    __syncthreads();
    tc_fence_after();
    pdl_wait();
    const uint32_t tmem_base = *reinterpret_cast<volatile uint32_t*>(smem + ScoreSmem::tmem_ptr);

    const int nt = prm.nt;
    const size_t hl = (size_t)prm.H * nt * kTile;
    const bool elide = (PASS == 2) && prm.n_keys != nullptr;
    const CUtensorMap* a_maps = (PASS == 1) ? maps.q : (elide ? maps.kc : maps.k);
    const CUtensorMap* b_maps = (PASS == 1) ? maps.k : maps.q;
    const int a_l1 = (PASS == 1) ? prm.q_dim1_is_l : (elide ? prm.kc_dim1_is_l : prm.k_dim1_is_l);
    const int b_l1 = (PASS == 1) ? prm.k_dim1_is_l : prm.q_dim1_is_l;
    TileRange range(prm.H, prm.Hl, nt, elide ? prm.n_keys : nullptr);
    int ul, tb0, tb1;

    if (warp == 0) {
        if (lane == 0) {
            uint32_t cnt = 0, ucnt = 0;
            while (range.next(ul, tb0, tb1)) {
                const int layer = range.layer;
                const int h = ul / range.nta, ta = (ul - h * range.nta) * kPair;
                const int hh = layer * prm.Hl + h;
                const int nt_a = range.nt_a;
                const CUtensorMap* a_map = a_maps + layer;
                const CUtensorMap* b_map = b_maps + layer;
                const int a_head = (PASS == 1) ? h : h / prm.G;
                const int b_head = (PASS == 1) ? h / prm.G : h;
                const int as = ucnt % kASlots;
                mbar_wait_feeder(a_empty(as), ((ucnt / kASlots) & 1u) ^ 1u);
                mbar_arrive_expect_tx(a_full(as), kPair * prm.n_atoms * kHalfBytes);
                for (int pa = 0; pa < kPair; ++pa)
                    for (int kk = 0; kk < prm.n_atoms; ++kk) {
                        const int row = ((ta + pa < nt_a) ? ta + pa : ta) * kTile;
                        tma_load_3d(base + ScoreSmem::a_tile + (as * kPair + pa) * kTileBytes + kk * kHalfBytes, a_map, kk * 64,
                                    a_l1 ? row : a_head, a_l1 ? a_head : row, a_full(as));
                    }
                ++ucnt;
                for (int tb = tb0; tb < tb1; ++tb, ++cnt) {
                    const int s = cnt % kStages;
                    mbar_wait_feeder(b_empty(s), ((cnt / kStages) & 1u) ^ 1u);
                    mbar_arrive_expect_tx(b_full(s), prm.n_atoms * kHalfBytes);
                    const uint32_t dst = base + ScoreSmem::b_ring + s * kTileBytes;
                    for (int kk = 0; kk < prm.n_atoms; ++kk) {
                        const int row = tb * kTile;
                        tma_load_3d(dst + kk * kHalfBytes, b_map, kk * 64, b_l1 ? row : b_head, b_l1 ? b_head : row,
                                    b_full(s));
                    }
                    if (PASS == 2) {
                        const int sl = cnt % kStatSlots;
                        mbar_arrive_expect_tx(st_full(sl), kTile * 4u);
                        bulk_g2s(base + ScoreSmem::stats + sl * kTile * 4u,
                                 prm.stats + (size_t)hh * nt * kTile + (size_t)tb * kTile, kTile * 4u, st_full(sl));
                    }
                }
            }
        }
    } else if (warp == 1) {
        uint32_t cnt = 0, ucnt = 0;
        while (range.next(ul, tb0, tb1)) {
            const int as = ucnt % kASlots;
            mbar_wait_feeder(a_full(as), (ucnt / kASlots) & 1u);
            ++ucnt;
            for (int tb = tb0; tb < tb1; ++tb, ++cnt) {
                const int s = cnt % kStages, bp = 2 * (int)(cnt & 1u);
                mbar_wait_feeder(b_full(s), (cnt / kStages) & 1u);
                mbar_wait_feeder(t_empty(bp), ((cnt >> 1) & 1u) ^ 1u);
                mbar_wait_feeder(t_empty(bp + 1), ((cnt >> 1) & 1u) ^ 1u);
                tc_fence_after();
                if (elect_one()) {
                    const uint32_t b0 = base + ScoreSmem::b_ring + s * kTileBytes;
                    const int nks = prm.n_atoms * 4;
#pragma unroll
                    for (int pa = 0; pa < 2; ++pa) {
                        const uint32_t a0 = base + ScoreSmem::a_tile + (as * 2 + pa) * kTileBytes;
#pragma unroll 8
                        for (int ks = 0; ks < nks; ++ks) {
                            const uint32_t off = (ks >> 2) * kHalfBytes + (ks & 3) * 32;
                            umma_bf16(tmem_base + (bp + pa) * kTile, umma_desc_sw128(a0 + off), umma_desc_sw128(b0 + off), kIdesc,
                                      ks > 0 ? 1u : 0u);
                        }
                        tc_commit(t_full(bp + pa));
                    }
                    tc_commit(b_empty(s));
                    if (tb == tb1 - 1) tc_commit(a_empty(as));
                }
                __syncwarp();
            }
        }
    } else {
        const int sw = warp - 2;
        const int grp = sw >> 2;
        const int quarter = warp & 3;
        const int row = quarter * 32 + lane;
        const int half = grp & 1;
        const uint32_t lane_addr = tmem_base + ((uint32_t)(quarter * 32) << 16) + half * 64;
        float* merge = reinterpret_cast<float*>(smem + ScoreSmem::merge);
        const float inv = prm.inv_sqrt_d;
        const uint64_t inv2 = pk2(inv, inv), l2e2 = pk2(kLog2e, kLog2e);
        uint32_t cnt = 0;
        while (range.next(ul, tb0, tb1)) {
            const int hl_ = ul / range.nta, ta = (ul - hl_ * range.nta) * 2 + (grp >> 1);
            const int h = range.layer * prm.Hl + hl_;
            const bool has_tile = ta < range.nt_a;
            SoftmaxState st;
            for (int tb = tb0; tb < tb1; ++tb, ++cnt) {
                const int b = 2 * (int)(cnt & 1u) + (grp >> 1);
                mbar_wait(t_full(b), (cnt >> 1) & 1u);
                tc_fence_after();
                if (PASS == 2) mbar_wait(st_full(cnt % kStatSlots), (cnt / kStatSlots) & 1u);
                const int valid = prm.L - tb * kTile - half * 64;
                const float* cq = reinterpret_cast<const float*>(smem + ScoreSmem::stats) + (cnt % kStatSlots) * kTile + half * 64;
                if (has_tile) {
                    uint32_t r[64];
                    tmem_ld64(lane_addr + b * kTile, r);
                    tmem_ld_wait();
                    softmax_cols<PASS>(r, valid, st, cq, inv, inv2, l2e2);
                }
                tc_fence_before();
                __syncwarp();
                if (lane == 0) mbar_arrive(t_empty(b));
            }
            const float m = st.m;
            float a0, a1;
            upk2(st.acc, a0, a1);
            if (PASS == 2) { a0 = st.c0; a1 = st.c1; }
            const bool first = (tb0 == 0), last = (tb1 == nt);
            const int part = first ? 0 : (last ? 2 : 1);
            const bool fill1 = first && (last || range.next_cta_reaches_end_of(ul)), fill2 = first && last;
            const size_t o = (size_t)h * nt * kTile + (size_t)ta * kTile + row;
            const int g_lo = grp & ~1;
            const bool folder = (grp == g_lo) && has_tile;
            if (PASS == 1) {
                merge[(grp * kTile + row) * 2] = m;
                merge[(grp * kTile + row) * 2 + 1] = a0 + a1;
                asm volatile("bar.sync 1, %0;" ::"n"(kSoftmaxWarps * 32) : "memory");
                if (folder) {
                    float mn = -INFINITY;
                    for (int g = g_lo; g < g_lo + 2; ++g) mn = fmaxf(mn, merge[(g * kTile + row) * 2]);
                    float lt = 0.f;
                    for (int g = g_lo; g < g_lo + 2; ++g) {
                        const float mg = merge[(g * kTile + row) * 2];
                        if (mg > -INFINITY) lt += merge[(g * kTile + row) * 2 + 1] * ex2f((mg - mn) * kLog2e);
                    }
                    prm.ml_part[(size_t)part * hl + o] = make_float2(mn, lt);
                    if (fill1) prm.ml_part[hl + o] = make_float2(-INFINITY, 0.f);
                    if (fill2) prm.ml_part[2 * hl + o] = make_float2(-INFINITY, 0.f);
                }
                asm volatile("bar.sync 1, %0;" ::"n"(kSoftmaxWarps * 32) : "memory");
            } else {
                merge[grp * kTile + row] = a0 + a1;
                asm volatile("bar.sync 1, %0;" ::"n"(kSoftmaxWarps * 32) : "memory");
                if (folder) {
                    const float cs = merge[g_lo * kTile + row] + merge[(g_lo + 1) * kTile + row];
                    prm.colsum_part[(size_t)part * hl + o] = cs;
                    if (fill1) prm.colsum_part[hl + o] = 0.f;
                    if (fill2) prm.colsum_part[2 * hl + o] = 0.f;
                }
                asm volatile("bar.sync 1, %0;" ::"n"(kSoftmaxWarps * 32) : "memory");
            }
        }
    }
    tc_fence_before();
    __syncthreads();
    if (warp == 1) tmem_dealloc(tmem_base, 512);
}

__global__ void pivot_stats_merge_kernel(const float2* __restrict__ ml_part, int H, int L, int Lpad, float* __restrict__ stats) {
    pdl_enter();
    const int q = blockIdx.x * blockDim.x + threadIdx.x;
    const int h = blockIdx.y;
    if (q >= Lpad) return;
    const size_t o = (size_t)h * Lpad + q, hl = (size_t)H * Lpad;
    const float2 p0 = ml_part[o], p1 = ml_part[hl + o], p2 = ml_part[2 * hl + o];
    const float mn = fmaxf(fmaxf(p0.x, p1.x), p2.x);
    float lt = 0.f;
    if (p0.x > -INFINITY) lt += p0.y * ex2f((p0.x - mn) * kLog2e);
    if (p1.x > -INFINITY) lt += p1.y * ex2f((p1.x - mn) * kLog2e);
    if (p2.x > -INFINITY) lt += p2.y * ex2f((p2.x - mn) * kLog2e);
    stats[o] = (q < L) ? fmaf(mn, kLog2e, lg2f(lt)) : INFINITY;
}

struct HeadScoreOut {
    __nv_bfloat16* p[kMaxBatchLayers];
    const int32_t* slot[kMaxBatchLayers];
    int KVH;
};

__global__ void pivot_head_reduce_kernel(const float* __restrict__ colsum_part, int H, int G, int L, int Lpad,
                                         const __grid_constant__ HeadScoreOut out) {
    pdl_enter();
    const int k = blockIdx.x * blockDim.x + threadIdx.x;
    const int g = blockIdx.y;
    if (k >= L) return;
    const size_t hl = (size_t)H * Lpad;
    const int layer = g / out.KVH;
    int col = k;
    if (out.slot[layer]) {
        col = out.slot[layer][k];
        if (col < 0) {
            out.p[layer][(size_t)(g - layer * out.KVH) * L + k] = __float2bfloat16_rn(1.0f);
            return;
        }
    }
    float v[4] = {0.f, 0.f, 0.f, 0.f};
    for (int j = 0; j < G; ++j) {
        const size_t o = (size_t)(g * G + j) * Lpad + col;
        v[j & 3] += round_bf16((colsum_part[o] + colsum_part[hl + o]) + colsum_part[2 * hl + o]);
    }
    const float s = ((v[0] + v[1]) + v[2]) + v[3];
    out.p[layer][(size_t)(g - layer * out.KVH) * L + k] = __float2bfloat16_rn(s * (1.0f / (float)G));
}

typedef CUresult (*EncodeTiledFn)(CUtensorMap*, CUtensorMapDataType, cuuint32_t, void*, const cuuint64_t*, const cuuint64_t*,
                                  const cuuint32_t*, const cuuint32_t*, CUtensorMapInterleave, CUtensorMapSwizzle,
                                  CUtensorMapL2promotion, CUtensorMapFloatOOBfill);

static EncodeTiledFn get_encode_fn() {
    static EncodeTiledFn fn = nullptr;
    if (fn) return fn;
    void* p = nullptr;
    cudaDriverEntryPointQueryResult qres;
    if (cudaGetDriverEntryPoint("cuTensorMapEncodeTiled", &p, cudaEnableDefault, &qres) != cudaSuccess ||
        qres != cudaDriverEntryPointSuccess)
        return nullptr;
    fn = reinterpret_cast<EncodeTiledFn>(p);
    return fn;
}

static int make_map(CUtensorMap* map, const void* ptr, int64_t heads, int64_t L, int64_t D, int64_t stride_h,
                    int64_t stride_l, int* dim1_is_l) {
    EncodeTiledFn enc = get_encode_fn();
    if (!enc) return RTK_E_DRIVER;
    const bool l_first = (heads == 1) || (stride_l <= stride_h);
    *dim1_is_l = l_first ? 1 : 0;
    cuuint64_t dims[3] = {(cuuint64_t)D, (cuuint64_t)(l_first ? L : heads), (cuuint64_t)(l_first ? heads : L)};
    cuuint64_t strides[2] = {(cuuint64_t)((l_first ? stride_l : stride_h) * 2), (cuuint64_t)((l_first ? stride_h : stride_l) * 2)};
    if (heads == 1) strides[1] = (cuuint64_t)(stride_l * 2) * (cuuint64_t)L;
    cuuint32_t box[3] = {64u, (cuuint32_t)(l_first ? kTile : 1), (cuuint32_t)(l_first ? 1 : kTile)};
    cuuint32_t estr[3] = {1u, 1u, 1u};
    CUresult r = enc(map, CU_TENSOR_MAP_DATA_TYPE_BFLOAT16, 3, const_cast<void*>(ptr), dims, strides, box, estr,
                     CU_TENSOR_MAP_INTERLEAVE_NONE, CU_TENSOR_MAP_SWIZZLE_128B, CU_TENSOR_MAP_L2_PROMOTION_L2_256B,
                     CU_TENSOR_MAP_FLOAT_OOB_FILL_NONE);
    return r == CUDA_SUCCESS ? 0 : RTK_E_DRIVER;
}

}

using namespace rtk;

extern "C" size_t rtk_pivot_score_workspace_bytes(int64_t H, int64_t L) {
    if (H < 1 || L < 1) return 0;
    const size_t lpad = (size_t)((L + kTile - 1) / kTile) * kTile;
    return 10 * (size_t)H * lpad * sizeof(float);
}

namespace rtk {

template <int NL>
static int score_launch(const ScoreBatch& b, ScoreParams prm, cudaStream_t st) {
    ScoreMaps<NL> maps;
    for (int l = 0; l < b.n; ++l) {
        int ql = 0, kl = 0;
        int rc = make_map(&maps.q[l], b.q[l], b.H, b.L, b.D, b.q_stride_h[l], b.q_stride_l[l], &ql);
        if (rc) return rc;
        rc = make_map(&maps.k[l], b.k[l], b.KVH, b.L, b.D, b.k_stride_h[l], b.k_stride_l[l], &kl);
        if (rc) return rc;
        if (l == 0) { prm.q_dim1_is_l = ql; prm.k_dim1_is_l = kl; }
        else if (ql != prm.q_dim1_is_l || kl != prm.k_dim1_is_l) return RTK_E_UNSUPPORTED;
        if (prm.n_keys) {
            int cl = 0;
            rc = make_map(&maps.kc[l], b.kc[l], b.KVH, b.L, b.D, b.D, b.KVH * b.D, &cl);
            if (rc) return rc;
            prm.kc_dim1_is_l = cl;
        } else {
            maps.kc[l] = maps.k[l];
        }
    }
    for (int l = b.n; l < NL; ++l) { maps.q[l] = maps.q[0]; maps.k[l] = maps.k[0]; maps.kc[l] = maps.kc[0]; }
    int dev = 0, sms = 0;
    cudaGetDevice(&dev);
    cudaDeviceGetAttribute(&sms, cudaDevAttrMultiProcessorCount, dev);
    const int units = prm.Hl * ((prm.nt + kPair - 1) / kPair);
    const long long gmax = (long long)units * prm.nt / ((prm.nt + 1) / 2);
    const int grid = (int)(gmax < sms ? (gmax < 1 ? 1 : gmax) : sms);
    const size_t smem = ScoreSmem::total + 1024;
    cudaError_t e = cudaFuncSetAttribute(pivot_score_kernel<1, NL>, cudaFuncAttributeMaxDynamicSharedMemorySize, (int)smem);
    if (e != cudaSuccess) return (int)e;
    e = cudaFuncSetAttribute(pivot_score_kernel<2, NL>, cudaFuncAttributeMaxDynamicSharedMemorySize, (int)smem);
    if (e != cudaSuccess) return (int)e;
    HeadScoreOut out;
    out.KVH = (int)b.KVH;
    for (int l = 0; l < kMaxBatchLayers; ++l) {
        out.p[l] = reinterpret_cast<__nv_bfloat16*>(b.head_scores[l < b.n ? l : 0]);
        out.slot[l] = prm.n_keys ? b.slot[l < b.n ? l : 0] : nullptr;
    }
    RTK_LAUNCH_PDL((pivot_score_kernel<1, NL>), grid, kScoreThreads2, smem, st, maps, prm);
    dim3 g1((unsigned)((prm.nt * kTile + 255) / 256), (unsigned)prm.H);
    RTK_LAUNCH_PDL(pivot_stats_merge_kernel, g1, 256, 0, st, prm.ml_part, prm.H, prm.L, prm.nt * kTile, prm.stats);
    RTK_LAUNCH_PDL((pivot_score_kernel<2, NL>), grid, kScoreThreads2, smem, st, maps, prm);
    dim3 g2((unsigned)((prm.L + 255) / 256), (unsigned)(b.KVH * b.n));
    RTK_LAUNCH_PDL(pivot_head_reduce_kernel, g2, 256, 0, st, prm.colsum_part, prm.H, prm.G, prm.L, prm.nt * kTile, out);
    return 0;
}

int pivot_score_batch(const ScoreBatch& b, void* workspace, size_t workspace_bytes, cudaStream_t st) {
    if (b.n < 1 || b.n > kMaxBatchLayers || !workspace || b.H < 1 || b.KVH < 1 || b.L < 1) return RTK_E_BADARG;
    if ((b.D != 64 && b.D != 128) || b.H % b.KVH != 0 || b.L > 16384 || b.H > 256) return RTK_E_UNSUPPORTED;
    if (((uintptr_t)workspace & 15u) != 0) return RTK_E_ALIGN;
    for (int l = 0; l < b.n; ++l) {
        if (!b.q[l] || !b.k[l] || !b.head_scores[l]) return RTK_E_BADARG;
        if ((((uintptr_t)b.q[l] | (uintptr_t)b.k[l]) & 15u) != 0) return RTK_E_ALIGN;
        if ((b.q_stride_h[l] | b.q_stride_l[l] | b.k_stride_h[l] | b.k_stride_l[l]) % 8 != 0) return RTK_E_ALIGN;
    }
    if (workspace_bytes < rtk_pivot_score_workspace_bytes(b.H * b.n, b.L)) return RTK_E_WORKSPACE;

    ScoreParams prm;
    prm.H = (int)(b.H * b.n);
    prm.Hl = (int)b.H;
    prm.G = (int)(b.H / b.KVH);
    prm.L = (int)b.L;
    prm.nt = (int)((b.L + kTile - 1) / kTile);
    prm.n_atoms = (int)(b.D / 64);
    prm.q_dim1_is_l = prm.k_dim1_is_l = prm.kc_dim1_is_l = 0;
    prm.n_keys = b.n_keys;
    if (b.n_keys)
        for (int l = 0; l < b.n; ++l)
            if (!b.kc[l] || !b.slot[l] || ((uintptr_t)b.kc[l] & 15u) != 0) return RTK_E_BADARG;
    const float sq = (float)sqrt((double)b.D);
    prm.inv_sqrt_d = 1.0f / sq;
    const size_t plane = (size_t)prm.H * prm.nt * kTile;
    prm.ml_part = reinterpret_cast<float2*>(workspace);
    prm.stats = reinterpret_cast<float*>(workspace) + 6 * plane;
    prm.colsum_part = prm.stats + plane;
    return b.n == 1 ? score_launch<1>(b, prm, st) : score_launch<kMaxBatchLayers>(b, prm, st);
}

}

extern "C" int rtk_pivot_score(const void* q, int64_t H, int64_t q_stride_h, int64_t q_stride_l, const void* k, int64_t KVH,
                               int64_t k_stride_h, int64_t k_stride_l, int64_t L, int64_t D, void* head_scores,
                               void* workspace, size_t workspace_bytes, void* stream) {
    RTK_NVTX("rtk_pivot_score");
    if (!q || !k || !head_scores || !workspace || H < 1 || KVH < 1 || L < 1) return RTK_E_BADARG;
    ScoreBatch b = {};
    b.n = 1; b.H = H; b.KVH = KVH; b.L = L; b.D = D;
    b.q[0] = q; b.k[0] = k; b.head_scores[0] = head_scores;
    b.q_stride_h[0] = q_stride_h; b.q_stride_l[0] = q_stride_l; b.k_stride_h[0] = k_stride_h; b.k_stride_l[0] = k_stride_l;
    return pivot_score_batch(b, workspace, workspace_bytes, (cudaStream_t)stream);
}
```

video-retake_b200/csrc/rtk_common.cuh:

```cuda
#pragma once

#include <cuda_bf16.h>
#include <cuda_runtime.h>
#include <nvtx3/nvToolsExt.h>
#include <stdint.h>

#include "../../include/rtk_b200.h"

namespace rtk {

extern long long g_launches;

#define RTK_CHECK_LAUNCH()                                   \
    do {                                                     \
        ++::rtk::g_launches;                                 \
        cudaError_t e__ = cudaGetLastError();                \
        if (e__ != cudaSuccess) return (int)e__;             \
    } while (0)

constexpr int kWarp = 32;

struct NvtxRange {
    explicit NvtxRange(const char* name) { nvtxRangePushA(name); }
    ~NvtxRange() { nvtxRangePop(); }
    NvtxRange(const NvtxRange&) = delete;
    NvtxRange& operator=(const NvtxRange&) = delete;
};
#define RTK_NVTX(name) ::rtk::NvtxRange nvtx_range__(name)

struct DisAux {
    float* sim;
    float* nrm;
    long long si, sp;
};
int dpselect_sim_nrm(const void* x, int64_t T, int64_t N, int64_t C, DisAux aux, cudaStream_t st);

constexpr int kMaxBatchLayers = 32;
struct ScoreBatch {
    int n;
    int64_t H, KVH, L, D;
    const void* q[kMaxBatchLayers];
    const void* k[kMaxBatchLayers];
    void* head_scores[kMaxBatchLayers];
    int64_t q_stride_h[kMaxBatchLayers], q_stride_l[kMaxBatchLayers], k_stride_h[kMaxBatchLayers], k_stride_l[kMaxBatchLayers];
    const void* kc[kMaxBatchLayers];
    const int32_t* slot[kMaxBatchLayers];
    const int32_t* n_keys;
};
int pivot_score_batch(const ScoreBatch& b, void* workspace, size_t workspace_bytes, cudaStream_t st);

__device__ __forceinline__ void pdl_trigger() { asm volatile("griddepcontrol.launch_dependents;" ::: "memory"); }
__device__ __forceinline__ void pdl_wait() { asm volatile("griddepcontrol.wait;" ::: "memory"); }
#ifndef RTK_PDL_EARLY_SMALL
#define RTK_PDL_EARLY_SMALL 1
#endif
#ifndef RTK_PDL_EARLY_SCORE
#define RTK_PDL_EARLY_SCORE 1
#endif
__device__ __forceinline__ void pdl_enter() {
    if (RTK_PDL_EARLY_SMALL) pdl_trigger();
    pdl_wait();
}

bool pdl_enabled();

template <typename... KArgs, typename... Args>
static inline cudaError_t launch_pdl(void (*kern)(KArgs...), dim3 grid, dim3 block, size_t smem, cudaStream_t st,
                                     Args&&... args) {
    cudaLaunchConfig_t cfg = {};
    cfg.gridDim = grid;
    cfg.blockDim = block;
    cfg.dynamicSmemBytes = smem;
    cfg.stream = st;
    cudaLaunchAttribute attr[1];
    attr[0].id = cudaLaunchAttributeProgrammaticStreamSerialization;
    attr[0].val.programmaticStreamSerializationAllowed = 1;
    cfg.attrs = attr;
    cfg.numAttrs = pdl_enabled() ? 1 : 0;
    return cudaLaunchKernelEx(&cfg, kern, static_cast<KArgs>(args)...);
}
#define RTK_LAUNCH_PDL(kern, grid, block, smem, st, ...)                                                  \
    do {                                                                                                  \
        ++::rtk::g_launches;                                                                              \
        cudaError_t le__ = ::rtk::launch_pdl(kern, dim3(grid), dim3(block), (size_t)(smem), st, __VA_ARGS__); \
        if (le__ != cudaSuccess) return (int)le__;                                                        \
    } while (0)

__device__ __forceinline__ float bf16lo_to_f32(uint32_t packed) { return __uint_as_float(packed << 16); }
__device__ __forceinline__ float bf16hi_to_f32(uint32_t packed) { return __uint_as_float(packed & 0xffff0000u); }

__device__ __forceinline__ uint32_t pack_bf16x2_rn(float lo, float hi) {
    uint32_t d;
    asm("cvt.rn.bf16x2.f32 %0, %1, %2;" : "=r"(d) : "f"(hi), "f"(lo));
    return d;
}
__device__ __forceinline__ float round_bf16(float x) {
    return __bfloat162float(__float2bfloat16_rn(x));
}
__device__ __forceinline__ uint32_t mul_bf16x2_rn(uint32_t a, uint32_t b) {
    uint32_t d;
    asm("mul.rn.bf16x2 %0, %1, %2;" : "=r"(d) : "r"(a), "r"(b));
    return d;
}

__device__ __forceinline__ void fma_sq_bf16x2(float& acc_lo, float& acc_hi, uint32_t p) {
    asm("{\n\t.reg .b16 lo, hi;\n\t"
        "mov.b32 {lo, hi}, %2;\n\t"
        "fma.rn.f32.bf16 %0, lo, lo, %0;\n\t"
        "fma.rn.f32.bf16 %1, hi, hi, %1;\n\t}"
        : "+f"(acc_lo), "+f"(acc_hi)
        : "r"(p));
}
__device__ __forceinline__ void add_bf16x2(float& acc_lo, float& acc_hi, uint32_t p) {
    asm("{\n\t.reg .b16 lo, hi;\n\t"
        "mov.b32 {lo, hi}, %2;\n\t"
        "add.rn.f32.bf16 %0, lo, %0;\n\t"
        "add.rn.f32.bf16 %1, hi, %1;\n\t}"
        : "+f"(acc_lo), "+f"(acc_hi)
        : "r"(p));
}
__device__ __forceinline__ uint32_t scale_bf16x2_rn(uint32_t p, float s) {
    return pack_bf16x2_rn(bf16lo_to_f32(p) * s, bf16hi_to_f32(p) * s);
}

__device__ __forceinline__ uint32_t f32_to_ordered(float v) {
    uint32_t x = __float_as_uint(v);
    uint32_t mask = (x & 0x80000000u) ? 0xffffffffu : 0x80000000u;
    return (v == v) ? (x ^ mask) : 0xffffffffu;
}

__device__ __forceinline__ uint32_t smem_u32(const void* p) { return (uint32_t)__cvta_generic_to_shared(p); }

__device__ __forceinline__ void mbar_init(uint32_t bar, uint32_t count) {
    asm volatile("mbarrier.init.shared::cta.b64 [%0], %1;" ::"r"(bar), "r"(count) : "memory");
}
__device__ __forceinline__ void fence_mbar_init() {
    asm volatile("fence.mbarrier_init.release.cluster;" ::: "memory");
}
__device__ __forceinline__ void fence_proxy_async() {
    asm volatile("fence.proxy.async.shared::cta;" ::: "memory");
}
__device__ __forceinline__ void mbar_arrive_expect_tx(uint32_t bar, uint32_t bytes) {
    asm volatile("mbarrier.arrive.expect_tx.shared::cta.b64 _, [%0], %1;" ::"r"(bar), "r"(bytes) : "memory");
}
__device__ __forceinline__ void mbar_arrive(uint32_t bar) {
    asm volatile("mbarrier.arrive.shared::cta.b64 _, [%0];" ::"r"(bar) : "memory");
}
__device__ __forceinline__ bool mbar_try_wait(uint32_t bar, uint32_t parity) {
    uint32_t ok;
    asm volatile(
        "{\n\t.reg .pred p;\n\t"
        "mbarrier.try_wait.parity.shared::cta.b64 p, [%1], %2;\n\t"
        "selp.u32 %0, 1, 0, p;\n\t}"
        : "=r"(ok)
        : "r"(bar), "r"(parity)
        : "memory");
    return ok != 0;
}
__device__ __forceinline__ void mbar_wait(uint32_t bar, uint32_t parity) {
    while (!mbar_try_wait(bar, parity)) {
    }
}
__device__ __forceinline__ void bulk_g2s(uint32_t dst_smem, const void* src, uint32_t bytes, uint32_t bar) {
    asm volatile("cp.async.bulk.shared::cluster.global.mbarrier::complete_tx::bytes [%0], [%1], %2, [%3];" ::"r"(dst_smem),
                 "l"(src), "r"(bytes), "r"(bar)
                 : "memory");
}
__device__ __forceinline__ void bulk_s2g(void* dst, uint32_t src_smem, uint32_t bytes) {
    asm volatile("cp.async.bulk.global.shared::cta.bulk_group [%0], [%1], %2;" ::"l"(dst), "r"(src_smem), "r"(bytes)
                 : "memory");
}
__device__ __forceinline__ void bulk_commit() { asm volatile("cp.async.bulk.commit_group;" ::: "memory"); }
template <int N>
__device__ __forceinline__ void bulk_wait_read() {
    asm volatile("cp.async.bulk.wait_group.read %0;" ::"n"(N) : "memory");
}
template <int N>
__device__ __forceinline__ void bulk_wait_all() {
    asm volatile("cp.async.bulk.wait_group %0;" ::"n"(N) : "memory");
}

__device__ __forceinline__ bool elect_one() {
    uint32_t pred;
    asm volatile(
        "{\n\t.reg .pred p;\n\t"
        "elect.sync _|p, 0xffffffff;\n\t"
        "selp.u32 %0, 1, 0, p;\n\t}"
        : "=r"(pred));
    return pred != 0;
}

}
```

video-retake_b200/retake/_native.py:

```python
from __future__ import annotations

import ctypes as C
import os

import torch

_HERE = os.path.dirname(os.path.abspath(__file__))
LIB_PATH = os.environ.get("RTK_B200_LIB", os.path.join(os.path.dirname(_HERE), "lib", "librtk_b200.so"))

_lib = None
ABI_VERSION = 3


class RtkError(RuntimeError):
    pass


def lib() -> C.CDLL:
    global _lib
    if _lib is not None:
        return _lib
    if not os.path.exists(LIB_PATH):
        raise RtkError(
            f"{LIB_PATH} not found: build it with `python video-retake_b200/build.py` "
            "(nvcc, sm_100a). There is no CPU or stock-PyTorch fallback for this path."
        )
    L = C.CDLL(LIB_PATH)
    p, i64, i32, f32, sz = C.c_void_p, C.c_int64, C.c_int, C.c_float, C.c_size_t
    sig = {
        "rtk_version": ([], C.c_int),
        "rtk_build_id": ([], C.c_char_p),
        "rtk_debug_key_elision": ([i32], C.c_int),
        "rtk_error_string": ([C.c_int], C.c_char_p),
        "rtk_launch_count": ([], i64),
        "rtk_dpselect_dis": ([p, i64, i64, i64, i32, p, p], C.c_int),
        "rtk_dpselect_select": ([p, i64, i64, i64, i32, p, p, p], C.c_int),
        "rtk_dpselect_gather": ([p, i64, i64, i64, p, i64, i32, p, p], C.c_int),
        "rtk_gather_rows": ([p, i64, p, i64, p, p], C.c_int),
        "rtk_dpselect_keyframe": ([p, i64, i64, i64, i64, i32, p, p, p, p, p], C.c_int),
        "rtk_dpselect_gather_owned": ([p, i64, i64, i64, i64, i64, i64, p, i64, i32, p, p], C.c_int),
        "rtk_mallm_workspace_bytes": ([i64, i64, i64, i32], sz),
        "rtk_mallm_compress": ([p, p, i64, i64, i64, i64, i32, i32, p, p, p, sz, p], C.c_int),
        "rtk_pivot_rope": ([p, i64, i64, i64, i64, i64, p, p, i32, p, f32, i32, p, i64, i64, p], C.c_int),
        "rtk_pivot_score_workspace_bytes": ([i64, i64], sz),
        "rtk_pivot_score": ([p, i64, i64, i64, p, i64, i64, i64, i64, i64, p, p, sz, p], C.c_int),
        "rtk_pivot_select": ([p, i64, i64, p, i64, p, p, p], C.c_int),
        "rtk_pivot_compact": ([p, p, i64, i64, i64, i64, i64, p, i64, p, p, i64, p, i32, p, i32, p], C.c_int),
        "rtk_pivot_rope_tables": ([p, i32, i64, i64, p, p, f32, p, p, p], C.c_int),
        "rtk_pivot_update_workspace_bytes": ([i64, i64, i64, i64], sz),
        "rtk_pivot_update": ([p, p], C.c_int),
        "rtk_pivot_update_batch_workspace_bytes": ([i64, i64, i64, i64, i64], sz),
        "rtk_pivot_update_batch": ([p, i64, p, sz, p], C.c_int),
        "rtk_kv_block_copy": ([i32, p, p, p, p, p, p, p, p, i64, p], C.c_int),
    }
    for name, (args, res) in sig.items():
        fn = getattr(L, name)
        fn.argtypes, fn.restype = args, res
    if L.rtk_version() != ABI_VERSION:
        raise RtkError(f"ABI mismatch: library reports version {L.rtk_version()}, binding expects {ABI_VERSION}")
    _check_build_id(L)
    _lib = L
    return L


def _source_id():
    import importlib.util
    path = os.path.join(os.path.dirname(_HERE), "build.py")
    if not os.path.exists(path) or not os.path.isdir(os.path.join(os.path.dirname(_HERE), "csrc")):
        return None
    spec = importlib.util.spec_from_file_location("rtk_build_for_id", path)
    mod = importlib.util.module_from_spec(spec)
    spec.loader.exec_module(mod)
    return mod.source_id()


def _check_build_id(L) -> None:
    if "RTK_B200_LIB" in os.environ or os.environ.get("RTK_ALLOW_STALE_LIB") == "1":
        return
    want = _source_id()
    got = L.rtk_build_id().decode()
    if want is not None and got != want:
        raise RtkError(f"{LIB_PATH} was built from other sources (library id {got}, sources {want}): "
                       "run `python video-retake_b200/build.py`")


def build_id() -> str:
    return lib().rtk_build_id().decode()


EXPORTS = ("rtk_version", "rtk_build_id", "rtk_debug_key_elision", "rtk_error_string", "rtk_launch_count", "rtk_dpselect_dis", "rtk_dpselect_select",
           "rtk_dpselect_gather", "rtk_dpselect_keyframe", "rtk_gather_rows", "rtk_dpselect_gather_owned", "rtk_mallm_workspace_bytes", "rtk_mallm_compress", "rtk_pivot_rope", "rtk_pivot_score_workspace_bytes", "rtk_pivot_score",
           "rtk_pivot_select", "rtk_pivot_compact", "rtk_pivot_rope_tables", "rtk_pivot_update_workspace_bytes",
           "rtk_pivot_update", "rtk_pivot_update_batch_workspace_bytes", "rtk_pivot_update_batch", "rtk_kv_block_copy")


def check(rc: int, what: str) -> None:
    if rc != 0:
        raise RtkError(f"{what} failed: {lib().rtk_error_string(rc).decode()} (code {rc})")


def require_cuda(t: torch.Tensor, name: str, dtype=None) -> None:
    if not isinstance(t, torch.Tensor) or not t.is_cuda:
        raise RtkError(f"{name} must be a CUDA tensor: this path has no CPU implementation")
    if dtype is not None and t.dtype != dtype:
        raise TypeError(f"{name} must be {dtype}, got {t.dtype}")


def stream_ptr(device) -> int:
    return torch.cuda.current_stream(device).cuda_stream


def launch_count() -> int:
    return int(lib().rtk_launch_count())
```

Before: 3568.

## Fuse Q/K un-RoPE into pivot score kernel with cross-block layer counters

```diff
diff --git a/include/rtk_b200.h b/include/rtk_b200.h
--- a/include/rtk_b200.h
+++ b/include/rtk_b200.h
@@ -20,6 +20,7 @@
 const char* rtk_build_id(void);
 const char* rtk_error_string(int code);
 int         rtk_debug_key_elision(int on);
+int         rtk_debug_fused_unrope(int on);
 int64_t     rtk_launch_count(void);
 
 
diff --git a/video-retake_b200/csrc/pivot_misc.cu b/video-retake_b200/csrc/pivot_misc.cu
--- a/video-retake_b200/csrc/pivot_misc.cu
+++ b/video-retake_b200/csrc/pivot_misc.cu
@@ -1,21 +1,11 @@
+#include <atomic>
 #include <climits>
 
 #include <stdlib.h>
 
-#include "rtk_common.cuh"
+#include "rtk_rope.cuh"
 
 namespace rtk {
-
-struct RopeParams {
-    int heads, L, D, n_pos, forward;
-    long long stride_h, stride_l, out_stride_h, out_stride_l;
-    int heads2;
-    const __nv_bfloat16* x2;
-    __nv_bfloat16* out2;
-    long long stride_h2, stride_l2, out_stride_h2, out_stride_l2;
-    int bound[6];
-    float inv_scale2;
-};
 
 static bool mrope_bounds(int n_pos, const int32_t* sec, int64_t D, int bound[6]) {
     int acc = 0;
@@ -24,13 +14,6 @@
         bound[i] = acc;
     }
     return n_pos != 3 || acc == D;
-}
-
-__device__ __forceinline__ int rope_pos_row(const RopeParams& p, int c) {
-    if (p.n_pos == 1) return 0;
-    int i = 0;
-    while (i < 5 && c >= p.bound[i]) ++i;
-    return i % 3;
 }
 
 __global__ void __launch_bounds__(256)
@@ -65,40 +48,10 @@
     ob = __float2bfloat16_rn(yb);
 }
 
-__device__ __forceinline__ void rope_table_entry(const RopeParams& p, const float* __restrict__ inv_freq, const long long* pv,
-                                                 int c, float scaling, float& co, float& si) {
-    const int half = p.D >> 1;
-    const float ang = inv_freq[c < half ? c : c - half] * (float)pv[rope_pos_row(p, c)];
-    co = __bfloat162float(__float2bfloat16_rn(cosf(ang) * scaling));
-    si = __bfloat162float(__float2bfloat16_rn(sinf(ang) * scaling));
-}
-
 #ifndef RTK_UNROPE_TOK
 #define RTK_UNROPE_TOK 2
 #endif
 constexpr int kUnropeTok = RTK_UNROPE_TOK;
-
-__device__ __forceinline__ uint32_t sub_bf16x2_rn(uint32_t a, uint32_t b) {
-    uint32_t d;
-    asm("sub.rn.bf16x2 %0, %1, %2;" : "=r"(d) : "r"(a), "r"(b));
-    return d;
-}
-__device__ __forceinline__ uint32_t add_bf16x2_rn(uint32_t a, uint32_t b) {
-    uint32_t d;
-    asm("add.rn.bf16x2 %0, %1, %2;" : "=r"(d) : "r"(a), "r"(b));
-    return d;
-}
-__device__ __forceinline__ void unrotate_bf16x2(uint32_t xa, uint32_t xb, uint32_t cs, uint32_t sn, bool scale, float inv_scale2,
-                                                uint32_t& oa, uint32_t& ob) {
-    const uint32_t ta = mul_bf16x2_rn(xa, cs), ra = mul_bf16x2_rn(xb ^ 0x80008000u, sn);
-    const uint32_t tb = mul_bf16x2_rn(xb, cs), rb = mul_bf16x2_rn(xa, sn);
-    oa = sub_bf16x2_rn(ta, ra);
-    ob = sub_bf16x2_rn(tb, rb);
-    if (scale) {
-        oa = scale_bf16x2_rn(oa, inv_scale2);
-        ob = scale_bf16x2_rn(ob, inv_scale2);
-    }
-}
 
 __device__ __forceinline__ void unrope_qk_body(const __nv_bfloat16* __restrict__ x, const long long* __restrict__ pos,
                                                const float* __restrict__ inv_freq, float scaling,
@@ -155,10 +108,7 @@
                 const uint4 cs = *reinterpret_cast<const uint4*>(&s_cos[t][c0]);
                 const uint4 sn = *reinterpret_cast<const uint4*>(&s_sin[t][c0]);
                 uint4 ol4, oh4;
-                unrotate_bf16x2(a4.x, b4.x, cs.x, sn.x, scale, p.inv_scale2, ol4.x, oh4.x);
-                unrotate_bf16x2(a4.y, b4.y, cs.y, sn.y, scale, p.inv_scale2, ol4.y, oh4.y);
-                unrotate_bf16x2(a4.z, b4.z, cs.z, sn.z, scale, p.inv_scale2, ol4.z, oh4.z);
-                unrotate_bf16x2(a4.w, b4.w, cs.w, sn.w, scale, p.inv_scale2, ol4.w, oh4.w);
+                unrotate_vec(a4, b4, cs, sn, scale, p.inv_scale2, ol4, oh4);
                 *reinterpret_cast<uint4*>(dst + c0) = ol4;
                 *reinterpret_cast<uint4*>(dst + c0 + half) = oh4;
             }
@@ -319,12 +269,14 @@
     }
 }
 
-static int key_elide_prepare(KeyElide& ke, int n, ScoreBatch& sb, cudaStream_t st) {
+static int key_elide_prepare(KeyElide& ke, int n, bool gather, ScoreBatch& sb, cudaStream_t st) {
     RTK_LAUNCH_PDL(pivot_keymask_scan_kernel, (unsigned)n, 1024, 0, st, ke);
-    const long long total = (long long)ke.L * ke.KVH * (ke.D >> 3);
-    long long gx = (total + 255) / 256;
-    if (gx > 148 * 8) gx = 148 * 8;
-    RTK_LAUNCH_PDL(pivot_keys_compact_kernel, dim3((unsigned)gx, (unsigned)n), 256, 0, st, ke);
+    if (gather) {
+        const long long total = (long long)ke.L * ke.KVH * (ke.D >> 3);
+        long long gx = (total + 255) / 256;
+        if (gx > 148 * 8) gx = 148 * 8;
+        RTK_LAUNCH_PDL(pivot_keys_compact_kernel, dim3((unsigned)gx, (unsigned)n), 256, 0, st, ke);
+    }
     for (int i = 0; i < n; ++i) {
         sb.kc[i] = ke.kc[i];
         sb.slot[i] = ke.slot[i];
@@ -441,11 +393,6 @@
     uint32_t v;
     asm volatile("ld.acquire.sys.global.u32 %0, [%1];" : "=r"(v) : "l"(p) : "memory");
     return v;
-}
-__device__ __forceinline__ unsigned long long globaltimer_ns() {
-    unsigned long long t;
-    asm volatile("mov.u64 %0, %%globaltimer;" : "=l"(t));
-    return t;
 }
 __device__ __forceinline__ void xchg_wait(const uint32_t* flags, int n, uint32_t epoch, unsigned long long timeout_ns) {
     if ((int)threadIdx.x < n) {
@@ -675,6 +622,7 @@
     }();
     return ns;
 }
+static std::atomic<int> g_fused_unrope{1};
 bool pdl_enabled() {
     static const bool on = [] {
         const char* e = getenv("RTK_NO_PDL");
@@ -692,6 +640,12 @@
 extern "C" int rtk_debug_key_elision(int on) {
     const int prev = rtk::key_elision_enabled() ? 1 : 0;
     if (on >= 0) rtk::g_key_elision = on ? 1 : 0;
+    return prev;
+}
+
+extern "C" int rtk_debug_fused_unrope(int on) {
+    const int prev = rtk::g_fused_unrope.load();
+    if (on >= 0) rtk::g_fused_unrope.store(on ? 1 : 0);
     return prev;
 }
 
@@ -807,7 +761,7 @@
     const size_t n = (size_t)(n_layers < kMaxBatchLayers ? n_layers : kMaxBatchLayers);
     return align256(rtk_pivot_score_workspace_bytes(H * (int64_t)n, L)) +
            n * (align256((size_t)H * L * D * 2) + align256((size_t)KVH * L * D * 2)) + align256(n * sizeof(long long)) + 256 +
-           n * key_elide_bytes(KVH, L, D) + 256;
+           n * key_elide_bytes(KVH, L, D) + 256 + align256(n * sizeof(unsigned long long));
 }
 
 extern "C" size_t rtk_pivot_update_workspace_bytes(int64_t H, int64_t KVH, int64_t L, int64_t D) {
@@ -830,7 +784,8 @@
     long long* tmin = (long long*)ws;   ws += align256((size_t)n * sizeof(long long)) + 256;
     char* kc0 = ws;                     ws += (size_t)n * align256((size_t)KVH * L * D * 2);
     char* slot0 = ws;                   ws += (size_t)n * align256((size_t)L * 4);
-    int32_t* nkeys_ws = (int32_t*)ws;
+    int32_t* nkeys_ws = (int32_t*)ws;   ws += 256;
+    unsigned long long* unrope_ctr = (unsigned long long*)ws;
 
     BatchLayers t = {};
     ScoreBatch sb = {};
@@ -867,7 +822,24 @@
     mrope_bounds(a0.n_pos, a0.mrope_section, D, rp.bound);
     const bool xchg = a0.xchg_world > 1;
     const int64_t score_rows = a0.score_rows > 0 ? a0.score_rows : KVH;
-    if (reforge && !a0.skip_score) {
+    const bool fused = reforge && !a0.skip_score && a0.inv_freq && g_fused_unrope.load() && pivot_score_fused_unrope_fits(H, L);
+    static std::atomic<uint32_t> epoch_src{0};
+    UnropeLayers un = {};
+    if (fused) {
+        uint32_t ep = ++epoch_src;
+        if (ep == 0) ep = ++epoch_src;
+        un.inv_freq = a0.inv_freq; un.scaling = a0.attention_scaling; un.inv_scale2 = a0.inv_scale2;
+        un.H = (int)H; un.KVH = (int)KVH; un.L = (int)L; un.D = (int)D; un.n_pos = a0.n_pos;
+        for (int i = 0; i < 6; ++i) un.bound[i] = rp.bound[i];
+        un.counters = unrope_ctr; un.epoch = ep; un.timeout_ns = xchg_timeout_ns();
+        for (int i = 0; i < n; ++i) {
+            un.q[i] = t.q[i]; un.q_stride_h[i] = t.q_stride_h[i]; un.q_stride_l[i] = t.q_stride_l[i];
+            un.k[i] = t.k_in[i]; un.k_stride_h[i] = t.kin_stride_h[i]; un.k_stride_l[i] = t.kin_stride_l[i];
+            un.pos[i] = t.pos[i]; un.qu[i] = t.qu[i]; un.ku[i] = t.ku[i];
+        }
+        sb.unrope = &un;
+    }
+    if (reforge && !a0.skip_score && !fused) {
         if (a0.inv_freq) {
             RTK_LAUNCH_PDL(pivot_unrope_qk_batch_kernel, dim3((unsigned)((L + kUnropeTok - 1) / kUnropeTok), (unsigned)n), 256, 0, st, t, a0.inv_freq,
                            a0.attention_scaling, rp);
@@ -891,8 +863,10 @@
                 ke.k[i] = t.k[j]; ke.k_stride_h[i] = t.k_stride_h[j]; ke.k_stride_l[i] = t.k_stride_l[j];
                 ke.kc[i] = (__nv_bfloat16*)(kc0 + (size_t)j * align256((size_t)KVH * L * D * 2));
             }
-            int rc = key_elide_prepare(ke, n, sb, st);
+            int rc = key_elide_prepare(ke, n, !fused, sb, st);
             if (rc) return rc;
+            if (fused)
+                for (int i = 0; i < n; ++i) { un.kc[i] = ke.kc[i]; un.slot[i] = ke.slot[i]; }
         }
         if (a0.ev_score_begin) cudaEventRecord((cudaEvent_t)a0.ev_score_begin, st);
         int rc = pivot_score_batch(sb, score_ws, rtk_pivot_score_workspace_bytes(H * n, L), st);
diff --git a/video-retake_b200/csrc/pivot_score.cu b/video-retake_b200/csrc/pivot_score.cu
--- a/video-retake_b200/csrc/pivot_score.cu
+++ b/video-retake_b200/csrc/pivot_score.cu
@@ -1,6 +1,9 @@
 #include <cuda.h>
-
-#include "rtk_common.cuh"
+#include <string.h>
+
+#include <atomic>
+
+#include "rtk_rope.cuh"
 
 namespace rtk {
 
@@ -22,7 +25,9 @@
     static constexpr uint32_t bars = merge + 4 * kTile * 2 * 4;
     static constexpr uint32_t n_bars = 4 + 2 * kStages + 2 * kAccBufs + kStatSlots;
     static constexpr uint32_t tmem_ptr = bars + n_bars * 8;
-    static constexpr uint32_t total = tmem_ptr + 16;
+    static constexpr uint32_t prod_layer = tmem_ptr + 4;
+    static constexpr uint32_t rope = tmem_ptr + 16;
+    static constexpr uint32_t total = rope + 2 * kRopeTok * 64 * 2;
 };
 
 __device__ __forceinline__ void tmem_alloc(uint32_t smem_dst, uint32_t ncols) {
@@ -100,6 +105,7 @@
 struct ScoreMaps {
     CUtensorMap q[NL], k[NL];
     CUtensorMap kc[NL];
+    UnropeLayers un;
 };
 
 struct ScoreParams {
@@ -254,10 +260,18 @@
 constexpr int kGroups = 4;
 constexpr int kSoftmaxWarps = 4 * kGroups;
 constexpr int kScoreThreads2 = (2 + kSoftmaxWarps) * 32;
+#ifndef RTK_UNROPE_WARPS
+#define RTK_UNROPE_WARPS 2
+#endif
+#ifndef RTK_UNROPE_AHEAD
+#define RTK_UNROPE_AHEAD 1
+#endif
+constexpr int kUnropeWarps = RTK_UNROPE_WARPS;
+constexpr int kScoreThreads1 = kScoreThreads2 + kUnropeWarps * 32;
 constexpr int kTileArrivals = 8;
 
 template <int PASS, int NL>
-__global__ void __launch_bounds__(kScoreThreads2, 1)
+__global__ void __launch_bounds__(PASS == 1 ? kScoreThreads1 : kScoreThreads2, 1)
 pivot_score_kernel(const __grid_constant__ ScoreMaps<NL> maps, ScoreParams prm) {
     if (RTK_PDL_EARLY_SCORE) pdl_trigger();
     extern __shared__ __align__(1024) uint8_t smem_raw[];
@@ -280,6 +294,7 @@
         for (int b = 0; b < kAccBufs; ++b) { mbar_init(t_full(b), 1); mbar_init(t_empty(b), kTileArrivals); }
         for (int i = 0; i < kStatSlots; ++i) mbar_init(st_full(i), 1);
         fence_mbar_init();
+        *reinterpret_cast<volatile int*>(smem + ScoreSmem::prod_layer) = -1;
     }
     if (warp == 1) tmem_alloc(base + ScoreSmem::tmem_ptr, 512);
     tc_fence_before();
@@ -287,6 +302,16 @@
     tc_fence_after();
     pdl_wait();
     const uint32_t tmem_base = *reinterpret_cast<volatile uint32_t*>(smem + ScoreSmem::tmem_ptr);
+    const bool fused = (PASS == 1) && maps.un.counters != nullptr;
+    const int ut0 = (int)((unsigned)prm.L * blockIdx.x / gridDim.x), ut1 = (int)((unsigned)prm.L * (blockIdx.x + 1) / gridDim.x);
+    __nv_bfloat16* s_cos = reinterpret_cast<__nv_bfloat16*>(smem + ScoreSmem::rope);
+    __nv_bfloat16* s_sin = s_cos + kRopeTok * 64;
+    if (fused) {
+        unrope_tokens(maps.un, 0, ut0, ut1, threadIdx.x, blockDim.x, 2, s_cos, s_sin);
+        fence_proxy_async_global();
+        __syncthreads();
+        if (threadIdx.x == 0) unrope_arrive(maps.un.counters, maps.un.epoch);
+    }
 
     const int nt = prm.nt;
     const size_t hl = (size_t)prm.H * nt * kTile;
@@ -301,8 +326,15 @@
     if (warp == 0) {
         if (lane == 0) {
             uint32_t cnt = 0, ucnt = 0;
+            int ready = -1;
             while (range.next(ul, tb0, tb1)) {
                 const int layer = range.layer;
+                if (fused && layer > ready) {
+                    for (int l = ready + 1; l <= layer; ++l)
+                        unrope_wait(maps.un.counters + l, maps.un.epoch, gridDim.x, maps.un.timeout_ns);
+                    ready = layer;
+                    *reinterpret_cast<volatile int*>(smem + ScoreSmem::prod_layer) = layer;
+                }
                 const int h = ul / range.nta, ta = (ul - h * range.nta) * kPair;
                 const int hh = layer * prm.Hl + h;
                 const int nt_a = range.nt_a;
@@ -369,6 +401,17 @@
                     if (tb == tb1 - 1) tc_commit(a_empty(as));
                 }
                 __syncwarp();
+            }
+        }
+    } else if (warp >= 2 + kSoftmaxWarps) {
+        if (fused) {
+            const int tid = threadIdx.x - (2 + kSoftmaxWarps) * 32;
+            for (int l = 1; l < range.n_layers; ++l) {
+                while (*reinterpret_cast<volatile int*>(smem + ScoreSmem::prod_layer) < l - RTK_UNROPE_AHEAD) __nanosleep(256);
+                unrope_tokens(maps.un, l, ut0, ut1, tid, kUnropeWarps * 32, 3, s_cos, s_sin);
+                fence_proxy_async_global();
+                named_bar_sync(3, kUnropeWarps * 32);
+                if (tid == 0) unrope_arrive(maps.un.counters + l, maps.un.epoch);
             }
         }
     } else {
@@ -540,6 +583,43 @@
 
 namespace rtk {
 
+constexpr size_t kScoreSmem = ScoreSmem::total + 1024;
+
+static int score_grid(int Hl, int nt) {
+    int dev = 0, sms = 0;
+    cudaGetDevice(&dev);
+    cudaDeviceGetAttribute(&sms, cudaDevAttrMultiProcessorCount, dev);
+    const int units = Hl * ((nt + kPair - 1) / kPair);
+    const long long gmax = (long long)units * nt / ((nt + 1) / 2);
+    return (int)(gmax < sms ? (gmax < 1 ? 1 : gmax) : sms);
+}
+
+template <int NL>
+static cudaError_t score_set_smem() {
+    cudaError_t e = cudaFuncSetAttribute(pivot_score_kernel<1, NL>, cudaFuncAttributeMaxDynamicSharedMemorySize, (int)kScoreSmem);
+    if (e != cudaSuccess) return e;
+    return cudaFuncSetAttribute(pivot_score_kernel<2, NL>, cudaFuncAttributeMaxDynamicSharedMemorySize, (int)kScoreSmem);
+}
+
+bool pivot_score_fused_unrope_fits(int64_t H, int64_t L) {
+    static std::atomic<int> per_sm_of[64];
+    int dev = 0, sms = 0;
+    cudaGetDevice(&dev);
+    std::atomic<int>& cached = per_sm_of[dev & 63];
+    int per_sm = cached.load();
+    if (per_sm == 0) {
+        int a = 0, b = 0;
+        const bool ok = score_set_smem<kMaxBatchLayers>() == cudaSuccess && score_set_smem<1>() == cudaSuccess &&
+                        cudaOccupancyMaxActiveBlocksPerMultiprocessor(&a, pivot_score_kernel<1, kMaxBatchLayers>, kScoreThreads1, kScoreSmem) == cudaSuccess &&
+                        cudaOccupancyMaxActiveBlocksPerMultiprocessor(&b, pivot_score_kernel<1, 1>, kScoreThreads1, kScoreSmem) == cudaSuccess;
+        per_sm = ok && (a < b ? a : b) > 0 ? (a < b ? a : b) : -1;
+        cached.store(per_sm);
+    }
+    if (per_sm < 0) return false;
+    cudaDeviceGetAttribute(&sms, cudaDevAttrMultiProcessorCount, dev);
+    return (long long)per_sm * sms >= score_grid((int)H, (int)((L + kTile - 1) / kTile));
+}
+
 template <int NL>
 static int score_launch(const ScoreBatch& b, ScoreParams prm, cudaStream_t st) {
     ScoreMaps<NL> maps;
@@ -561,16 +641,10 @@
         }
     }
     for (int l = b.n; l < NL; ++l) { maps.q[l] = maps.q[0]; maps.k[l] = maps.k[0]; maps.kc[l] = maps.kc[0]; }
-    int dev = 0, sms = 0;
-    cudaGetDevice(&dev);
-    cudaDeviceGetAttribute(&sms, cudaDevAttrMultiProcessorCount, dev);
-    const int units = prm.Hl * ((prm.nt + kPair - 1) / kPair);
-    const long long gmax = (long long)units * prm.nt / ((prm.nt + 1) / 2);
-    const int grid = (int)(gmax < sms ? (gmax < 1 ? 1 : gmax) : sms);
-    const size_t smem = ScoreSmem::total + 1024;
-    cudaError_t e = cudaFuncSetAttribute(pivot_score_kernel<1, NL>, cudaFuncAttributeMaxDynamicSharedMemorySize, (int)smem);
-    if (e != cudaSuccess) return (int)e;
-    e = cudaFuncSetAttribute(pivot_score_kernel<2, NL>, cudaFuncAttributeMaxDynamicSharedMemorySize, (int)smem);
+    if (b.unrope) maps.un = *b.unrope;
+    else memset(&maps.un, 0, sizeof(maps.un));
+    const int grid = score_grid(prm.Hl, prm.nt);
+    cudaError_t e = score_set_smem<NL>();
     if (e != cudaSuccess) return (int)e;
     HeadScoreOut out;
     out.KVH = (int)b.KVH;
@@ -578,10 +652,10 @@
         out.p[l] = reinterpret_cast<__nv_bfloat16*>(b.head_scores[l < b.n ? l : 0]);
         out.slot[l] = prm.n_keys ? b.slot[l < b.n ? l : 0] : nullptr;
     }
-    RTK_LAUNCH_PDL((pivot_score_kernel<1, NL>), grid, kScoreThreads2, smem, st, maps, prm);
+    RTK_LAUNCH_PDL((pivot_score_kernel<1, NL>), grid, kScoreThreads1, kScoreSmem, st, maps, prm);
     dim3 g1((unsigned)((prm.nt * kTile + 255) / 256), (unsigned)prm.H);
     RTK_LAUNCH_PDL(pivot_stats_merge_kernel, g1, 256, 0, st, prm.ml_part, prm.H, prm.L, prm.nt * kTile, prm.stats);
-    RTK_LAUNCH_PDL((pivot_score_kernel<2, NL>), grid, kScoreThreads2, smem, st, maps, prm);
+    RTK_LAUNCH_PDL((pivot_score_kernel<2, NL>), grid, kScoreThreads2, kScoreSmem, st, maps, prm);
     dim3 g2((unsigned)((prm.L + 255) / 256), (unsigned)(b.KVH * b.n));
     RTK_LAUNCH_PDL(pivot_head_reduce_kernel, g2, 256, 0, st, prm.colsum_part, prm.H, prm.G, prm.L, prm.nt * kTile, out);
     return 0;
diff --git a/video-retake_b200/csrc/rtk_common.cuh b/video-retake_b200/csrc/rtk_common.cuh
--- a/video-retake_b200/csrc/rtk_common.cuh
+++ b/video-retake_b200/csrc/rtk_common.cuh
@@ -36,6 +36,7 @@
 int dpselect_sim_nrm(const void* x, int64_t T, int64_t N, int64_t C, DisAux aux, cudaStream_t st);
 
 constexpr int kMaxBatchLayers = 32;
+struct UnropeLayers;
 struct ScoreBatch {
     int n;
     int64_t H, KVH, L, D;
@@ -46,8 +47,10 @@
     const void* kc[kMaxBatchLayers];
     const int32_t* slot[kMaxBatchLayers];
     const int32_t* n_keys;
+    const UnropeLayers* unrope;
 };
 int pivot_score_batch(const ScoreBatch& b, void* workspace, size_t workspace_bytes, cudaStream_t st);
+bool pivot_score_fused_unrope_fits(int64_t H, int64_t L);
 
 __device__ __forceinline__ void pdl_trigger() { asm volatile("griddepcontrol.launch_dependents;" ::: "memory"); }
 __device__ __forceinline__ void pdl_wait() { asm volatile("griddepcontrol.wait;" ::: "memory"); }
diff --git a/video-retake_b200/csrc/rtk_rope.cuh b/video-retake_b200/csrc/rtk_rope.cuh
--- /dev/null
+++ b/video-retake_b200/csrc/rtk_rope.cuh
@@ -0,0 +1,197 @@
+#pragma once
+
+#include "rtk_common.cuh"
+
+namespace rtk {
+
+struct RopeParams {
+    int heads, L, D, n_pos, forward;
+    long long stride_h, stride_l, out_stride_h, out_stride_l;
+    int heads2;
+    const __nv_bfloat16* x2;
+    __nv_bfloat16* out2;
+    long long stride_h2, stride_l2, out_stride_h2, out_stride_l2;
+    int bound[6];
+    float inv_scale2;
+};
+
+__device__ __forceinline__ int rope_pos_row(const RopeParams& p, int c) {
+    if (p.n_pos == 1) return 0;
+    int i = 0;
+    while (i < 5 && c >= p.bound[i]) ++i;
+    return i % 3;
+}
+
+__device__ __forceinline__ void rope_table_entry(const RopeParams& p, const float* __restrict__ inv_freq, const long long* pv,
+                                                 int c, float scaling, float& co, float& si) {
+    const int half = p.D >> 1;
+    const float ang = inv_freq[c < half ? c : c - half] * (float)pv[rope_pos_row(p, c)];
+    co = __bfloat162float(__float2bfloat16_rn(cosf(ang) * scaling));
+    si = __bfloat162float(__float2bfloat16_rn(sinf(ang) * scaling));
+}
+
+__device__ __forceinline__ uint32_t sub_bf16x2_rn(uint32_t a, uint32_t b) {
+    uint32_t d;
+    asm("sub.rn.bf16x2 %0, %1, %2;" : "=r"(d) : "r"(a), "r"(b));
+    return d;
+}
+__device__ __forceinline__ uint32_t add_bf16x2_rn(uint32_t a, uint32_t b) {
+    uint32_t d;
+    asm("add.rn.bf16x2 %0, %1, %2;" : "=r"(d) : "r"(a), "r"(b));
+    return d;
+}
+__device__ __forceinline__ void unrotate_bf16x2(uint32_t xa, uint32_t xb, uint32_t cs, uint32_t sn, bool scale, float inv_scale2,
+                                                uint32_t& oa, uint32_t& ob) {
+    const uint32_t ta = mul_bf16x2_rn(xa, cs), ra = mul_bf16x2_rn(xb ^ 0x80008000u, sn);
+    const uint32_t tb = mul_bf16x2_rn(xb, cs), rb = mul_bf16x2_rn(xa, sn);
+    oa = sub_bf16x2_rn(ta, ra);
+    ob = sub_bf16x2_rn(tb, rb);
+    if (scale) {
+        oa = scale_bf16x2_rn(oa, inv_scale2);
+        ob = scale_bf16x2_rn(ob, inv_scale2);
+    }
+}
+__device__ __forceinline__ void unrotate_vec(const uint4& a, const uint4& b, const uint4& cs, const uint4& sn, bool scale,
+                                             float inv_scale2, uint4& oa, uint4& ob) {
+    unrotate_bf16x2(a.x, b.x, cs.x, sn.x, scale, inv_scale2, oa.x, ob.x);
+    unrotate_bf16x2(a.y, b.y, cs.y, sn.y, scale, inv_scale2, oa.y, ob.y);
+    unrotate_bf16x2(a.z, b.z, cs.z, sn.z, scale, inv_scale2, oa.z, ob.z);
+    unrotate_bf16x2(a.w, b.w, cs.w, sn.w, scale, inv_scale2, oa.w, ob.w);
+}
+
+__device__ __forceinline__ unsigned long long globaltimer_ns() {
+    unsigned long long t;
+    asm volatile("mov.u64 %0, %%globaltimer;" : "=l"(t));
+    return t;
+}
+unsigned long long xchg_timeout_ns();
+
+struct UnropeLayers {
+    const __nv_bfloat16* q[kMaxBatchLayers];
+    const __nv_bfloat16* k[kMaxBatchLayers];
+    long long q_stride_h[kMaxBatchLayers], q_stride_l[kMaxBatchLayers];
+    long long k_stride_h[kMaxBatchLayers], k_stride_l[kMaxBatchLayers];
+    const long long* pos[kMaxBatchLayers];
+    __nv_bfloat16* qu[kMaxBatchLayers];
+    __nv_bfloat16* ku[kMaxBatchLayers];
+    __nv_bfloat16* kc[kMaxBatchLayers];
+    const int32_t* slot[kMaxBatchLayers];
+    const float* inv_freq;
+    float scaling, inv_scale2;
+    int H, KVH, L, D, n_pos;
+    int bound[6];
+    unsigned long long* counters;
+    uint32_t epoch;
+    unsigned long long timeout_ns;
+};
+
+constexpr int kRopeTok = 8;
+
+__device__ __forceinline__ void named_bar_sync(int id, int nthr) {
+    asm volatile("bar.sync %0, %1;" ::"r"(id), "r"(nthr) : "memory");
+}
+
+__device__ __forceinline__ void unrope_tokens(const UnropeLayers& u, int layer, int t0, int t1, int tid, int nthr, int bar,
+                                              __nv_bfloat16* s_cos, __nv_bfloat16* s_sin) {
+    RopeParams p;
+    p.D = u.D; p.n_pos = u.n_pos;
+#pragma unroll
+    for (int i = 0; i < 6; ++i) p.bound[i] = u.bound[i];
+    const int half = u.D >> 1, vshift = u.D == 128 ? 3 : 2;
+    const int ntask = (u.H + u.KVH) << vshift;
+    const bool scale = u.inv_scale2 != 1.0f;
+    const long long* __restrict__ pos = u.pos[layer];
+    const int32_t* __restrict__ slot = u.slot[layer];
+    __nv_bfloat16* kc = u.kc[layer];
+    const int nsub = nthr >= ntask ? nthr / ntask : 1;
+    const int sub = nthr >= ntask ? tid / ntask : 0;
+    const int r0 = nthr >= ntask ? tid - sub * ntask : tid, rstride = nthr >= ntask ? ntask : nthr;
+    for (int l0 = t0; l0 < t1; l0 += kRopeTok) {
+        const int nl = min(kRopeTok, t1 - l0);
+        for (int e = tid; e < nl * half; e += nthr) {
+            const int t = e / half, c = e - t * half;
+            long long pv[3] = {0, 0, 0};
+            for (int r = 0; r < u.n_pos; ++r) pv[r] = pos[(size_t)r * u.L + l0 + t];
+            float co, si;
+            rope_table_entry(p, u.inv_freq, pv, c, u.scaling, co, si);
+            s_cos[t * 64 + c] = __float2bfloat16_rn(co);
+            s_sin[t * 64 + c] = __float2bfloat16_rn(si);
+        }
+        named_bar_sync(bar, nthr);
+        if (sub < nsub) {
+            for (int r = r0; r < ntask; r += rstride) {
+                const int h = r >> vshift, c0 = (r & ((1 << vshift) - 1)) * 8;
+                const bool isk = h >= u.H;
+                const int hk = h - u.H;
+                const __nv_bfloat16* src = isk ? u.k[layer] + hk * u.k_stride_h[layer] : u.q[layer] + h * u.q_stride_h[layer];
+                const long long sl = isk ? u.k_stride_l[layer] : u.q_stride_l[layer];
+                __nv_bfloat16* dst = isk ? u.ku[layer] + (size_t)hk * u.D : u.qu[layer] + (size_t)h * u.D;
+                const long long dl = (long long)(isk ? u.KVH : u.H) * u.D;
+                for (int tb = sub; tb < nl; tb += 4 * nsub) {
+                    uint4 a4[4], b4[4];
+                    int srow[4];
+#pragma unroll
+                    for (int j = 0; j < 4; ++j) {
+                        const int t = tb + j * nsub;
+                        if (t < nl) {
+                            const __nv_bfloat16* s = src + (l0 + t) * sl + c0;
+                            a4[j] = *reinterpret_cast<const uint4*>(s);
+                            b4[j] = *reinterpret_cast<const uint4*>(s + half);
+                            srow[j] = (isk && kc) ? slot[l0 + t] : -1;
+                        }
+                    }
+#pragma unroll
+                    for (int j = 0; j < 4; ++j) {
+                        const int t = tb + j * nsub;
+                        if (t < nl) {
+                            const uint4 cs = *reinterpret_cast<const uint4*>(s_cos + t * 64 + c0);
+                            const uint4 sn = *reinterpret_cast<const uint4*>(s_sin + t * 64 + c0);
+                            uint4 ol4, oh4;
+                            unrotate_vec(a4[j], b4[j], cs, sn, scale, u.inv_scale2, ol4, oh4);
+                            __nv_bfloat16* d = dst + (l0 + t) * dl + c0;
+                            *reinterpret_cast<uint4*>(d) = ol4;
+                            *reinterpret_cast<uint4*>(d + half) = oh4;
+                            if (srow[j] >= 0) {
+                                __nv_bfloat16* dc = kc + ((size_t)srow[j] * u.KVH + hk) * u.D + c0;
+                                *reinterpret_cast<uint4*>(dc) = ol4;
+                                *reinterpret_cast<uint4*>(dc + half) = oh4;
+                            }
+                        }
+                    }
+                }
+            }
+        }
+        named_bar_sync(bar, nthr);
+    }
+}
+
+__device__ __forceinline__ void fence_proxy_async_global() { asm volatile("fence.proxy.async.global;" ::: "memory"); }
+
+__device__ __forceinline__ void unrope_arrive(unsigned long long* counter, uint32_t epoch) {
+    __threadfence();
+    const unsigned long long tag = (unsigned long long)epoch << 32;
+    unsigned long long old = *reinterpret_cast<volatile unsigned long long*>(counter), assumed;
+    do {
+        assumed = old;
+        const unsigned long long nv = ((assumed & 0xffffffff00000000ull) == tag) ? assumed + 1 : tag + 1;
+        old = atomicCAS(counter, assumed, nv);
+    } while (old != assumed);
+}
+__device__ __forceinline__ unsigned long long ld_acquire_gpu_u64(const unsigned long long* p) {
+    unsigned long long v;
+    asm volatile("ld.acquire.gpu.global.u64 %0, [%1];" : "=l"(v) : "l"(p) : "memory");
+    return v;
+}
+__device__ __forceinline__ void unrope_wait(const unsigned long long* counter, uint32_t epoch, unsigned n, unsigned long long timeout_ns) {
+    const unsigned long long want = ((unsigned long long)epoch << 32) | n;
+    if (ld_acquire_gpu_u64(counter) != want) {
+        const unsigned long long t0 = globaltimer_ns();
+        while (ld_acquire_gpu_u64(counter) != want) {
+            __nanosleep(64);
+            if (timeout_ns && globaltimer_ns() - t0 > timeout_ns) __trap();
+        }
+    }
+    fence_proxy_async_global();
+}
+
+}
diff --git a/video-retake_b200/retake/_native.py b/video-retake_b200/retake/_native.py
--- a/video-retake_b200/retake/_native.py
+++ b/video-retake_b200/retake/_native.py
@@ -31,6 +31,7 @@
         "rtk_version": ([], C.c_int),
         "rtk_build_id": ([], C.c_char_p),
         "rtk_debug_key_elision": ([i32], C.c_int),
+        "rtk_debug_fused_unrope": ([i32], C.c_int),
         "rtk_error_string": ([C.c_int], C.c_char_p),
         "rtk_launch_count": ([], i64),
         "rtk_dpselect_dis": ([p, i64, i64, i64, i32, p, p], C.c_int),
@@ -88,7 +89,7 @@
     return lib().rtk_build_id().decode()
 
 
-EXPORTS = ("rtk_version", "rtk_build_id", "rtk_debug_key_elision", "rtk_error_string", "rtk_launch_count", "rtk_dpselect_dis", "rtk_dpselect_select",
+EXPORTS = ("rtk_version", "rtk_build_id", "rtk_debug_key_elision", "rtk_debug_fused_unrope", "rtk_error_string", "rtk_launch_count", "rtk_dpselect_dis", "rtk_dpselect_select",
            "rtk_dpselect_gather", "rtk_dpselect_keyframe", "rtk_gather_rows", "rtk_dpselect_gather_owned", "rtk_mallm_workspace_bytes", "rtk_mallm_compress", "rtk_pivot_rope", "rtk_pivot_score_workspace_bytes", "rtk_pivot_score",
            "rtk_pivot_select", "rtk_pivot_compact", "rtk_pivot_rope_tables", "rtk_pivot_update_workspace_bytes",
            "rtk_pivot_update", "rtk_pivot_update_batch_workspace_bytes", "rtk_pivot_update_batch", "rtk_kv_block_copy")
```

After: 3629 (median of 6 runs). 1.7% higher.
